# JOBR0/PerceiverIO_Pytorch

Measured on AMD Instinct MI355X. Metric: samples/sec PerceiverIO fwd (ImageNet-224, 512x1024 latents, 8 blocks x 6 self-attends), higher is better.
Workload: dtype f16; 1 GPU; imagenet224 ClassificationPerceiver (conv+Fourier prep -> encoder 3136x322->512x1024, 8x6 SA -> decoder 1000 queries -> final Linear), all rows computed; batch_per_gpu=32, global_batch=32, precision_policy=fp16x2w/fp16sd/fp16x2af, parallelism=dp1 (batch sharded, all-gather of logits), launch=one HIP graph replay per step

## Files before the change

include/pio_hip.h:

```cpp
#ifndef PIO_HIP_H
#define PIO_HIP_H

#include <stddef.h>
#include <stdint.h>

#ifdef __cplusplus
extern "C" {
#endif

#define PIO_VERSION 100

enum {
    PIO_OK = 0,
    PIO_E_SHAPE = -1,
    PIO_E_ALIGN = -2,
    PIO_E_ARCH = -3,
    PIO_E_WORKSPACE = -4,
    PIO_E_LAUNCH = -5,
    PIO_E_ARG = -6,
    PIO_E_RANGE = -7
};

enum { PIO_DT_F16 = 0, PIO_DT_BF16 = 1 };


typedef struct pio_linear_t {
    const void *w_hi;
    const void *w_lo;
    const float *bias;
    int32_t n;
    int32_t k;
    int32_t lo_row0;
} pio_linear_t;

typedef struct pio_layernorm_t {
    const float *gamma;
    const float *beta;
    int32_t c;
    float eps;
} pio_layernorm_t;

typedef struct pio_attention_t {
    pio_linear_t q, k, v, o;
    int32_t heads;
    int32_t dk, dv;
    int32_t dkp, dvp;
    int32_t q_in, k_in, v_in, out;
    int32_t dtype;
    int32_t act_split;
    pio_linear_t qk;
    pio_linear_t qkv;
    pio_linear_t kq, vo;
} pio_attention_t;

typedef struct pio_mlp_t {
    pio_linear_t fc1, fc2;
    int32_t in, hidden, out;
    int32_t dtype;
    int32_t act_split;
} pio_mlp_t;

typedef struct pio_ln_fold_t {
    pio_linear_t qkv;
    const float *qkv_c;
    pio_linear_t fc1;
    const float *fc1_c;
    int32_t *range_flag;
} pio_ln_fold_t;

typedef struct pio_self_attention_t {
    pio_layernorm_t ln1, ln2;
    pio_attention_t attn;
    pio_mlp_t mlp;
    pio_ln_fold_t fold;
} pio_self_attention_t;

typedef struct pio_cross_attention_t {
    pio_layernorm_t ln_q, ln_kv, ln2;
    pio_attention_t attn;
    pio_mlp_t mlp;
    int32_t use_query_residual;
} pio_cross_attention_t;

typedef struct pio_tensor3_t {
    const float *data;
    int64_t stride_b;
    int64_t stride_t;
    int32_t B, T, C;
} pio_tensor3_t;

int pio_version(void);
int pio_arch_ok(void);
const char *pio_error_string(int code);

#define PIO_PROF_CLASSES 9
int pio_prof_begin(int32_t max_records);
int pio_prof_end(double *ms, double *flops, double *bytes, int64_t *launches);

int pio_qk_logit_absmax(int32_t dtype, int32_t dkp, int32_t dk, const void *Q, const void *K, int32_t B, int32_t H,
                        int32_t Tq, int32_t Tk, int64_t ldq, int64_t ldk, int64_t sQb, int64_t sKb, const uint8_t *kv_mask,
                        const uint8_t *q_mask, const uint8_t *full_mask, float *absmax, void *stream);
int pio_logit_probe_begin(float *records, int32_t max_records);
int pio_logit_probe_end(void);

int pio_absmax16(int32_t dtype, const void *x, int64_t rows, int32_t cols, int64_t ld, int32_t batch, int64_t stride_b,
                 float *absmax, void *stream);
enum {
    PIO_RK_CAST = 0,
    PIO_RK_Q = 1,
    PIO_RK_K = 2,
    PIO_RK_V = 3,
    PIO_RK_ATTN = 4,
    PIO_RK_HIDDEN = 5,
    PIO_RK_STREAM = 6
};
enum { PIO_RP_ATTENTION = 0, PIO_RP_CROSS = 1, PIO_RP_STACK = 2, PIO_RP_DECODER = 3 };
int pio_range_probe_begin(float *records, int32_t max_records);
int pio_range_probe_mark(int32_t part);
int pio_range_probe_end(int32_t *parts, int32_t *kinds, int32_t cap);

int pio_ln_fold_enable(int on);

int pio_gemm_kernel_override(int which);

int pio_stream_create_cu_mask(void **stream, const uint32_t *mask, uint32_t words);
int pio_stream_destroy(void *stream);
int pio_set_cu_budget(int32_t n_cu);

int32_t pio_pad8(int32_t c);
int32_t pio_padc(int32_t c);
size_t pio_packed_weight_bytes(int32_t out, int32_t in, int32_t row_heads, int32_t col_heads);
int pio_pack_linear(const float *w, const float *bias, int32_t out, int32_t in, int64_t ldw,
                    int32_t row_heads, int32_t col_heads, void *dst_hi, void *dst_lo, float *dst_bias,
                    int32_t dst_row0, int32_t k_pad, int32_t dtype, void *stream);

int pio_layernorm_cast(const pio_tensor3_t *x, const pio_layernorm_t *ln, void *y, void *y_lo, int32_t c_pad,
                       int32_t dtype, void *stream);

int pio_layernorm_cast_cat(const pio_tensor3_t *x1, const pio_tensor3_t *x2, const pio_layernorm_t *ln, void *y,
                           void *y_lo, int32_t c_pad, int32_t dtype, void *stream);

int pio_bn_relu_maxpool_tokens(const float *x, const float *scale, const float *shift, float *y, int32_t B, int32_t C,
                               int32_t H, int32_t W, int32_t pad_top, int32_t pad_left, void *stream);

typedef struct pio_gemm_t {
    const void *A, *B;
    const void *A_lo, *B_lo;
    void *C;
    void *C_lo;
    int32_t M, N, K;
    int64_t lda, ldb, ldc;
    int32_t batch, nh;
    int64_t sAb, sAh, sBb, sBh, sCb, sCh;
    const float *bias;
    int32_t bias_mode;
    int32_t act;
    float alpha;
    const float *R;
    int64_t ldr, r_stride_b;
    int32_t r_rows_per_batch;
    int32_t out_f32;
    int32_t n_store;
    int32_t dtype;
    void *X16;
    int64_t ld16;
    float *row_part;
    const float *ln_part;
    const float *ln_c;
    float ln_eps;
    void *X16_lo;
    const void *R16_hi, *R16_lo;
    int32_t b_lo_n0;
    int32_t *range_flag;
    int32_t ln_slots;
    int32_t row_slot_w;
} pio_gemm_t;
int pio_gemm_nt(const pio_gemm_t *g, void *stream);

int pio_softmax_rows(const float *S, int64_t lds, void *P, void *P_lo, int64_t ldp, int32_t B, int32_t H,
                     int32_t Tq, int32_t Tk, float scale, const uint8_t *kv_mask, const uint8_t *q_mask,
                     const uint8_t *full_mask, const float *bias, int32_t dtype, void *stream);

int pio_flash_attention(int32_t dtype, int32_t dkp, int32_t dvp, int32_t dk, const void *Q, const void *K, const void *V,
                        void *O, int32_t B, int32_t H, int32_t Tq, int32_t Tk, int64_t ldq, int64_t ldk, int64_t ldv,
                        int64_t ldo, int64_t sQb, int64_t sKb, int64_t sVb, int64_t sOb, int32_t v_rowmajor, void *stream);

size_t pio_flash_attention_pair_workspace_bytes(int32_t dkp, int32_t dvp, int32_t B, int32_t H, int32_t Tq, int32_t Tk);
int pio_flash_attention_pair(int32_t dtype, int32_t dkp, int32_t dvp, int32_t dk, const void *Q, const void *Q_lo,
                             const void *K, const void *K_lo, const void *V, void *O, void *O_lo, int32_t B, int32_t H,
                             int32_t Tq, int32_t Tk, int64_t ldq, int64_t ldk, int64_t ldv, int64_t ldo, int64_t sQb,
                             int64_t sKb, int64_t sVb, int64_t sOb, int32_t v_rowmajor, const uint8_t *kv_mask,
                             const uint8_t *q_mask, int32_t core, void *workspace, size_t workspace_bytes, void *stream);

size_t pio_attention_workspace_bytes(const pio_attention_t *a, int32_t B, int32_t Tq, int32_t Tk);
int pio_attention_fwd(const pio_attention_t *a, const pio_tensor3_t *inputs_q, const pio_tensor3_t *inputs_k,
                      const pio_tensor3_t *inputs_v, const uint8_t *kv_mask, const uint8_t *q_mask,
                      const uint8_t *full_mask, const float *attention_bias, float *out, float *probs_out,
                      void *workspace, size_t workspace_bytes, void *stream);

size_t pio_mlp_workspace_bytes(const pio_mlp_t *m, int64_t rows);
int pio_mlp_fwd(const pio_mlp_t *m, const pio_tensor3_t *x, float *out, void *workspace,
                size_t workspace_bytes, void *stream);

typedef struct pio_call_opts_t {
    int32_t ln_fold;
    int32_t cu_budget;
} pio_call_opts_t;

size_t pio_self_attention_workspace_bytes(const pio_self_attention_t *s, int32_t B, int32_t N);
int pio_self_attention_fwd(const pio_self_attention_t *s, const pio_tensor3_t *x, const uint8_t *kv_mask,
                           const uint8_t *q_mask, const uint8_t *full_mask, const float *attention_bias,
                           float *out, float *probs_out, void *workspace, size_t workspace_bytes, void *stream);

int pio_self_attention_fwd_opts(const pio_self_attention_t *s, const pio_tensor3_t *x, const uint8_t *kv_mask,
                                const uint8_t *q_mask, const uint8_t *full_mask, const float *attention_bias,
                                float *out, float *probs_out, void *workspace, size_t workspace_bytes, void *stream,
                                const pio_call_opts_t *opts);

size_t pio_cross_attention_workspace_bytes(const pio_cross_attention_t *c, int32_t B, int32_t Tq, int32_t Tk);
int pio_cross_attention_fwd(const pio_cross_attention_t *c, const pio_tensor3_t *inputs_q,
                            const pio_tensor3_t *inputs_kv, const uint8_t *kv_mask, const uint8_t *q_mask,
                            const uint8_t *full_mask, const float *attention_bias, float *out, float *probs_out,
                            void *workspace, size_t workspace_bytes, void *stream);

size_t pio_encoder_workspace_bytes(const pio_cross_attention_t *cross, const pio_self_attention_t *layers,
                                   int32_t L, int32_t B, int32_t M, int32_t N);
int pio_encoder_fwd(const pio_cross_attention_t *cross, const pio_self_attention_t *layers, int32_t L,
                    int32_t num_blocks, const pio_tensor3_t *inputs, const pio_tensor3_t *latents,
                    const uint8_t *input_mask, float *out, void *workspace, size_t workspace_bytes,
                    void *stream);

int pio_encoder_fwd_split(const pio_cross_attention_t *cross, const pio_self_attention_t *layers, int32_t L,
                          int32_t num_blocks, const pio_tensor3_t *inputs, const pio_tensor3_t *inputs_tail,
                          const pio_tensor3_t *latents, const uint8_t *input_mask, float *out, void *workspace,
                          size_t workspace_bytes, void *stream);

int pio_encoder_fwd_blocks(const pio_cross_attention_t *cross, const pio_self_attention_t *layers, int32_t L,
                           int32_t num_blocks, int32_t per_block, const pio_tensor3_t *inputs,
                           const pio_tensor3_t *inputs_tail, const pio_tensor3_t *latents, const uint8_t *input_mask,
                           float *out, void *workspace, size_t workspace_bytes, void *stream);

int pio_encoder_fwd_opts(const pio_cross_attention_t *cross, const pio_self_attention_t *layers, int32_t L,
                         int32_t num_blocks, int32_t per_block, const pio_tensor3_t *inputs,
                         const pio_tensor3_t *inputs_tail, const pio_tensor3_t *latents, const uint8_t *input_mask,
                         float *out, void *workspace, size_t workspace_bytes, void *stream,
                         const pio_call_opts_t *opts);

size_t pio_decoder_workspace_bytes(const pio_cross_attention_t *cross, const pio_linear_t *final_layer,
                                   int32_t B, int32_t Q, int32_t N);
int pio_decoder_fwd(const pio_cross_attention_t *cross, const pio_linear_t *final_layer, int32_t final_out,
                    const pio_tensor3_t *query, const pio_tensor3_t *latents, const uint8_t *query_mask,
                    float *out, void *workspace, size_t workspace_bytes, void *stream);

size_t pio_decoder_qcache_bytes(const pio_cross_attention_t *cross, int32_t Bq, int32_t Q);
int pio_decoder_fwd_qcache(const pio_cross_attention_t *cross, const pio_linear_t *final_layer, int32_t final_out,
                           const pio_tensor3_t *query, const pio_tensor3_t *latents, const uint8_t *query_mask,
                           float *out, void *workspace, size_t workspace_bytes, void *stream, void *q16_hi,
                           void *q16_lo, int32_t q16_valid);

int pio_decoder_fwd_split(const pio_cross_attention_t *cross, const pio_linear_t *final_layer, int32_t final_out,
                          const pio_tensor3_t *query, const pio_tensor3_t *query_tail, const pio_tensor3_t *latents,
                          const uint8_t *query_mask, float *out, void *workspace, size_t workspace_bytes, void *stream);

#ifdef __cplusplus
}
#endif
#endif
```

perceiverio_pytorch_amd/_lib.py:

```python
from __future__ import annotations

import ctypes as C
import os
import subprocess

_HERE = os.path.dirname(os.path.abspath(__file__))
LIB_PATH = os.environ.get("PIO_LIB_PATH", os.path.join(_HERE, "libpio_hip.so"))
CSRC = os.path.join(_HERE, "csrc")

PIO_DT_F16 = 0
PIO_DT_BF16 = 1

PIO_OK = 0
_ERRORS = {-1: "PIO_E_SHAPE", -2: "PIO_E_ALIGN", -3: "PIO_E_ARCH", -4: "PIO_E_WORKSPACE", -5: "PIO_E_LAUNCH",
           -6: "PIO_E_ARG", -7: "PIO_E_RANGE"}


class PioError(RuntimeError):
    pass


class Linear(C.Structure):
    _fields_ = [("w_hi", C.c_void_p), ("w_lo", C.c_void_p), ("bias", C.c_void_p), ("n", C.c_int32), ("k", C.c_int32),
                ("lo_row0", C.c_int32)]


class LayerNorm(C.Structure):
    _fields_ = [("gamma", C.c_void_p), ("beta", C.c_void_p), ("c", C.c_int32), ("eps", C.c_float)]


class Attention(C.Structure):
    _fields_ = [("q", Linear), ("k", Linear), ("v", Linear), ("o", Linear), ("heads", C.c_int32),
                ("dk", C.c_int32), ("dv", C.c_int32), ("dkp", C.c_int32), ("dvp", C.c_int32),
                ("q_in", C.c_int32), ("k_in", C.c_int32), ("v_in", C.c_int32), ("out", C.c_int32), ("dtype", C.c_int32),
                ("act_split", C.c_int32), ("qk", Linear), ("qkv", Linear), ("kq", Linear), ("vo", Linear)]


class Mlp(C.Structure):
    _fields_ = [("fc1", Linear), ("fc2", Linear), ("in_", C.c_int32), ("hidden", C.c_int32), ("out", C.c_int32),
                ("dtype", C.c_int32), ("act_split", C.c_int32)]


class LnFold(C.Structure):
    _fields_ = [("qkv", Linear), ("qkv_c", C.c_void_p), ("fc1", Linear), ("fc1_c", C.c_void_p),
                ("range_flag", C.c_void_p)]


class SelfAttention(C.Structure):
    _fields_ = [("ln1", LayerNorm), ("ln2", LayerNorm), ("attn", Attention), ("mlp", Mlp), ("fold", LnFold)]


class CrossAttention(C.Structure):
    _fields_ = [("ln_q", LayerNorm), ("ln_kv", LayerNorm), ("ln2", LayerNorm), ("attn", Attention), ("mlp", Mlp),
                ("use_query_residual", C.c_int32)]


class Tensor3(C.Structure):
    _fields_ = [("data", C.c_void_p), ("stride_b", C.c_int64), ("stride_t", C.c_int64), ("B", C.c_int32),
                ("T", C.c_int32), ("C", C.c_int32)]


class CallOpts(C.Structure):
    _fields_ = [("ln_fold", C.c_int32), ("cu_budget", C.c_int32)]


class Gemm(C.Structure):
    _fields_ = [("A", C.c_void_p), ("B", C.c_void_p), ("A_lo", C.c_void_p), ("B_lo", C.c_void_p), ("C", C.c_void_p),
                ("C_lo", C.c_void_p),
                ("M", C.c_int32), ("N", C.c_int32), ("K", C.c_int32),
                ("lda", C.c_int64), ("ldb", C.c_int64), ("ldc", C.c_int64),
                ("batch", C.c_int32), ("nh", C.c_int32),
                ("sAb", C.c_int64), ("sAh", C.c_int64), ("sBb", C.c_int64), ("sBh", C.c_int64),
                ("sCb", C.c_int64), ("sCh", C.c_int64),
                ("bias", C.c_void_p), ("bias_mode", C.c_int32), ("act", C.c_int32), ("alpha", C.c_float),
                ("R", C.c_void_p), ("ldr", C.c_int64), ("r_stride_b", C.c_int64),
                ("r_rows_per_batch", C.c_int32), ("out_f32", C.c_int32), ("n_store", C.c_int32),
                ("dtype", C.c_int32),
                ("X16", C.c_void_p), ("ld16", C.c_int64), ("row_part", C.c_void_p), ("ln_part", C.c_void_p),
                ("ln_c", C.c_void_p), ("ln_eps", C.c_float),
                ("X16_lo", C.c_void_p), ("R16_hi", C.c_void_p), ("R16_lo", C.c_void_p), ("b_lo_n0", C.c_int32),
                ("range_flag", C.c_void_p), ("ln_slots", C.c_int32), ("row_slot_w", C.c_int32)]


P = C.POINTER
_vp, _i32, _i64, _sz, _f = C.c_void_p, C.c_int32, C.c_int64, C.c_size_t, C.c_float
SIGNATURES = {
    "pio_version": (C.c_int, []),
    "pio_arch_ok": (C.c_int, []),
    "pio_error_string": (C.c_char_p, [C.c_int]),
    "pio_prof_begin": (C.c_int, [_i32]),
    "pio_prof_end": (C.c_int, [P(C.c_double), P(C.c_double), P(C.c_double), P(C.c_int64)]),
    "pio_qk_logit_absmax": (C.c_int, [_i32, _i32, _i32, _vp, _vp, _i32, _i32, _i32, _i32, _i64, _i64, _i64, _i64, _vp, _vp,
                                      _vp, _vp, _vp]),
    "pio_logit_probe_begin": (C.c_int, [_vp, _i32]),
    "pio_logit_probe_end": (C.c_int, []),
    "pio_absmax16": (C.c_int, [_i32, _vp, _i64, _i32, _i64, _i32, _i64, _vp, _vp]),
    "pio_range_probe_begin": (C.c_int, [_vp, _i32]),
    "pio_range_probe_mark": (C.c_int, [_i32]),
    "pio_range_probe_end": (C.c_int, [P(_i32), P(_i32), _i32]),
    "pio_pad8": (_i32, [_i32]),
    "pio_padc": (_i32, [_i32]),
    "pio_gemm_kernel_override": (C.c_int, [C.c_int]),
    "pio_ln_fold_enable": (C.c_int, [C.c_int]),
    "pio_stream_create_cu_mask": (C.c_int, [P(_vp), P(C.c_uint32), C.c_uint32]),
    "pio_stream_destroy": (C.c_int, [_vp]),
    "pio_set_cu_budget": (C.c_int, [_i32]),
    "pio_packed_weight_bytes": (_sz, [_i32, _i32, _i32, _i32]),
    "pio_pack_linear": (C.c_int, [_vp, _vp, _i32, _i32, _i64, _i32, _i32, _vp, _vp, _vp, _i32, _i32, _i32, _vp]),
    "pio_layernorm_cast": (C.c_int, [P(Tensor3), P(LayerNorm), _vp, _vp, _i32, _i32, _vp]),
    "pio_layernorm_cast_cat": (C.c_int, [P(Tensor3), P(Tensor3), P(LayerNorm), _vp, _vp, _i32, _i32, _vp]),
    "pio_bn_relu_maxpool_tokens": (C.c_int, [_vp, _vp, _vp, _vp, _i32, _i32, _i32, _i32, _i32, _i32, _vp]),
    "pio_gemm_nt": (C.c_int, [P(Gemm), _vp]),
    "pio_softmax_rows": (C.c_int, [_vp, _i64, _vp, _vp, _i64, _i32, _i32, _i32, _i32, _f, _vp, _vp, _vp, _vp, _i32, _vp]),
    "pio_flash_attention": (C.c_int, [_i32, _i32, _i32, _i32, _vp, _vp, _vp, _vp, _i32, _i32, _i32, _i32, _i64, _i64, _i64,
                                      _i64, _i64, _i64, _i64, _i64, _i32, _vp]),
    "pio_flash_attention_pair_workspace_bytes": (_sz, [_i32, _i32, _i32, _i32, _i32, _i32]),
    "pio_flash_attention_pair": (C.c_int, [_i32, _i32, _i32, _i32, _vp, _vp, _vp, _vp, _vp, _vp, _vp, _i32, _i32, _i32, _i32,
                                           _i64, _i64, _i64, _i64, _i64, _i64, _i64, _i64, _i32, _vp, _vp, _i32, _vp, _sz,
                                           _vp]),
    "pio_attention_workspace_bytes": (_sz, [P(Attention), _i32, _i32, _i32]),
    "pio_attention_fwd": (C.c_int, [P(Attention), P(Tensor3), P(Tensor3), P(Tensor3), _vp, _vp, _vp, _vp, _vp, _vp,
                                    _vp, _sz, _vp]),
    "pio_mlp_workspace_bytes": (_sz, [P(Mlp), _i64]),
    "pio_mlp_fwd": (C.c_int, [P(Mlp), P(Tensor3), _vp, _vp, _sz, _vp]),
    "pio_self_attention_workspace_bytes": (_sz, [P(SelfAttention), _i32, _i32]),
    "pio_self_attention_fwd": (C.c_int, [P(SelfAttention), P(Tensor3), _vp, _vp, _vp, _vp, _vp, _vp, _vp, _sz, _vp]),
    "pio_self_attention_fwd_opts": (C.c_int, [P(SelfAttention), P(Tensor3), _vp, _vp, _vp, _vp, _vp, _vp, _vp, _sz, _vp,
                                              P(CallOpts)]),
    "pio_cross_attention_workspace_bytes": (_sz, [P(CrossAttention), _i32, _i32, _i32]),
    "pio_cross_attention_fwd": (C.c_int, [P(CrossAttention), P(Tensor3), P(Tensor3), _vp, _vp, _vp, _vp, _vp, _vp,
                                          _vp, _sz, _vp]),
    "pio_encoder_workspace_bytes": (_sz, [P(CrossAttention), P(SelfAttention), _i32, _i32, _i32, _i32]),
    "pio_encoder_fwd": (C.c_int, [P(CrossAttention), P(SelfAttention), _i32, _i32, P(Tensor3), P(Tensor3), _vp, _vp,
                                  _vp, _sz, _vp]),
    "pio_encoder_fwd_split": (C.c_int, [P(CrossAttention), P(SelfAttention), _i32, _i32, P(Tensor3), P(Tensor3),
                                        P(Tensor3), _vp, _vp, _vp, _sz, _vp]),
    "pio_encoder_fwd_blocks": (C.c_int, [P(CrossAttention), P(SelfAttention), _i32, _i32, _i32, P(Tensor3), P(Tensor3),
                                         P(Tensor3), _vp, _vp, _vp, _sz, _vp]),
    "pio_encoder_fwd_opts": (C.c_int, [P(CrossAttention), P(SelfAttention), _i32, _i32, _i32, P(Tensor3), P(Tensor3),
                                       P(Tensor3), _vp, _vp, _vp, _sz, _vp, P(CallOpts)]),
    "pio_decoder_workspace_bytes": (_sz, [P(CrossAttention), P(Linear), _i32, _i32, _i32]),
    "pio_decoder_fwd": (C.c_int, [P(CrossAttention), P(Linear), _i32, P(Tensor3), P(Tensor3), _vp, _vp, _vp, _sz,
                                  _vp]),
    "pio_decoder_qcache_bytes": (_sz, [P(CrossAttention), _i32, _i32]),
    "pio_decoder_fwd_qcache": (C.c_int, [P(CrossAttention), P(Linear), _i32, P(Tensor3), P(Tensor3), _vp, _vp, _vp, _sz,
                                         _vp, _vp, _vp, _i32]),
    "pio_decoder_fwd_split": (C.c_int, [P(CrossAttention), P(Linear), _i32, P(Tensor3), P(Tensor3), P(Tensor3), _vp, _vp, _vp,
                                        _sz, _vp]),
}

_lib = None


def build(verbose: bool = False) -> str:
    out = subprocess.run(["make", "-C", CSRC, "-j8"], capture_output=True, text=True)
    if verbose or out.returncode:
        print(out.stdout[-4000:])
        print(out.stderr[-4000:])
    if out.returncode:
        raise PioError("building libpio_hip.so failed")
    return LIB_PATH


def lib() -> C.CDLL:
    global _lib
    if _lib is None:
        if not os.path.exists(LIB_PATH):
            raise PioError(f"{LIB_PATH} is missing: run `python -c 'import __graft_entry__ as g; g.build()'` "
                           "(there is no CPU / eager fallback for the PerceiverIO hot path)")
        l = C.CDLL(LIB_PATH)
        for name, (res, args) in SIGNATURES.items():
            fn = getattr(l, name)
            fn.restype = res
            fn.argtypes = args
        _lib = l
    return _lib


def check(code: int, what: str = "") -> None:
    if code != PIO_OK:
        raise PioError(f"{what}: {_ERRORS.get(code, code)}")
```

perceiverio_pytorch_amd/csrc/pio_blocks.hip:

```cpp
#include "pio_internal.h"

namespace pio {

#define PIO_TRY(expr)                  \
    do {                               \
        int _e = (expr);               \
        if (_e != PIO_OK) return _e;   \
    } while (0)

#define PIO_RANGE(kind, dtype, ptr, rows, cols, ld, batch, stride_b, stream) \
    do {                                                                      \
        if (range_probe_active())                                             \
            PIO_TRY(range_probe_record(kind, dtype, ptr, rows, cols, ld, batch, stride_b, stream)); \
    } while (0)

struct Pair {
    void *hi = nullptr, *lo = nullptr;
};

static Pair take_pair(Carver &c, size_t elems, bool split) {
    Pair p;
    p.hi = c.take(elems * 2);
    p.lo = split ? c.take(elems * 2) : nullptr;
    return p;
}

struct Residual {
    const float *ptr = nullptr;
    int64_t ld = 0, stride_b = 0;
    int rows_per_batch = 0;
};

static inline int pitch4(int c) { return (c + 3) & ~3; }

static Residual residual_of(const pio_tensor3_t &t) {
    Residual r;
    r.ptr = t.data;
    r.ld = t.stride_t;
    r.stride_b = t.stride_b;
    r.rows_per_batch = t.T;
    return r;
}

static pio_gemm_t gemm_defaults(int dtype) {
    pio_gemm_t g = {};
    g.batch = 1;
    g.nh = 1;
    g.alpha = 1.f;
    g.dtype = dtype;
    return g;
}

struct LnFold {
    const float *in_part = nullptr;
    const pio_linear_t *w = nullptr;
    const float *c = nullptr;
    float eps = 0.f;
    void *out16 = nullptr;
    int64_t ld16 = 0;
    float *out_part = nullptr;
    void *out16_lo = nullptr;
    const void *res16_hi = nullptr, *res16_lo = nullptr;
    int32_t *range_flag = nullptr;
    int in_slots = 0, slot_w = 0;
};

static int linear_fwd(const pio_linear_t &lin_plain, int dtype, Pair x, int64_t rows, void *y, void *y_lo, bool out_f32,
                      int n_logical, int64_t ldc, int act, const Residual *res, hipStream_t s,
                      const LnFold *fold = nullptr, int n_store16 = 0) {
    const pio_linear_t &lin = (fold && fold->in_part) ? *fold->w : lin_plain;
    pio_gemm_t g = gemm_defaults(dtype);
    if (fold && fold->in_part) {
        g.ln_part = fold->in_part;
        g.ln_c = fold->c;
        g.ln_eps = fold->eps;
        g.ln_slots = fold->in_slots;
    }
    if (fold && fold->out16) {
        g.X16 = fold->out16;
        g.ld16 = fold->ld16;
        g.row_part = fold->out_part;
        g.X16_lo = fold->out16_lo;
        g.R16_hi = fold->res16_hi;
        g.R16_lo = fold->res16_lo;
        g.range_flag = fold->range_flag;
        g.row_slot_w = fold->slot_w;
    }
    g.A = x.hi;
    g.A_lo = x.lo;
    g.B = lin.w_hi;
    g.B_lo = lin.w_lo;
    g.b_lo_n0 = lin.w_lo ? lin.lo_row0 : 0;
    g.C = y;
    g.C_lo = y_lo;
    g.M = (int)rows;
    g.N = out_f32 ? n_logical : lin.n;
    if (out_f32 && (n_logical & 3) && ldc >= pitch4(n_logical) && lin.n >= pitch4(n_logical) &&
        !(res && res->ptr && res->ld < pitch4(n_logical)))
        g.N = pitch4(n_logical);
    g.K = lin.k;
    g.lda = lin.k;
    g.ldb = lin.k;
    g.ldc = ldc;
    g.bias = lin.bias;
    g.bias_mode = lin.bias ? 1 : 0;
    g.act = act;
    g.out_f32 = out_f32 ? 1 : 0;
    g.n_store = (!out_f32 && n_store16 > g.N) ? n_store16 : g.N;
    if (res && res->ptr && !(fold && fold->res16_hi)) {
        g.R = res->ptr;
        g.ldr = res->ld;
        g.r_stride_b = res->stride_b;
        g.r_rows_per_batch = res->rows_per_batch;
    }
    return gemm_nt_launch(g, s);
}

static int cast_pair(const pio_tensor3_t &x, const pio_layernorm_t *ln, Pair y, int c_pad, int dtype, hipStream_t s,
                     int range_kind = PIO_RK_CAST) {
    PIO_TRY(layernorm_cast_launch(x, ln, y.hi, y.lo, c_pad, dtype, s));
    PIO_RANGE(range_kind, dtype, y.hi, (int64_t)x.B * x.T, x.C, c_pad, 1, 0, s);
    return PIO_OK;
}

static const int64_t kScoreCapBytes = 1ll << 30;

struct ScoreChunks {
    int b_chunk;
    int q_chunk;
};
static ScoreChunks score_chunks(int B, int H, int Tq, int Tk) {
    const int64_t per_sample = (int64_t)H * Tq * (int64_t)Tk * 4;
    ScoreChunks c{B, Tq};
    if ((int64_t)B * per_sample <= kScoreCapBytes) return c;
    int64_t bc = kScoreCapBytes / (per_sample > 0 ? per_sample : 1);
    if (bc >= 1) {
        c.b_chunk = (int)bc;
        return c;
    }
    c.b_chunk = 1;
    int64_t qc = kScoreCapBytes / ((int64_t)H * Tk * 4);
    qc = qc / 128 * 128;
    c.q_chunk = (int)(qc < 128 ? 128 : qc);
    if (c.q_chunk > Tq) c.q_chunk = Tq;
    return c;
}

struct AttnScratch {
    Pair q16, k16, vt16, p16, o16;
    float *scores;
    void *xpart;
    void carve(Carver &c, const pio_attention_t &a, int Bq, int B, int Tq, int Tk, bool lean = false) {
        const int64_t ldq = (int64_t)a.heads * a.dkp, ldo = (int64_t)a.heads * a.dvp, tkp = pad8(Tk);
        const int64_t tkv = round_up(Tk, 32);
        const bool sp = a.act_split != 0;
        const AttnRoute plan = attn_plan(a, B, Bq, Tq, Tk, lean);
        q16 = take_pair(c, (size_t)Bq * Tq * ldq, sp);
        k16 = take_pair(c, (size_t)B * Tk * ldq, sp);
        vt16 = take_pair(c, (size_t)B * ldo * tkv, sp);
        scores = nullptr;
        p16 = Pair();
        if (plan.need_scores) {
            const ScoreChunks ch = score_chunks(B, a.heads, Tq, Tk);
            scores = (float *)c.take((size_t)ch.b_chunk * a.heads * ch.q_chunk * (int64_t)Tk * 4);
            p16 = take_pair(c, (size_t)ch.b_chunk * a.heads * ch.q_chunk * tkp, sp);
        }
        o16 = take_pair(c, (size_t)B * Tq * ldo, sp);
        xpart = plan.xpart_bytes ? c.take(plan.xpart_bytes) : nullptr;
    }
};

static int check_attention(const pio_attention_t &a) {
    if (a.heads <= 0 || a.dk <= 0 || a.dv <= 0) return PIO_E_SHAPE;
    if (a.dkp != pad8(a.dk) || a.dvp != pad8(a.dv)) return PIO_E_SHAPE;
    if (a.q.n != a.heads * a.dkp || a.k.n != a.heads * a.dkp || a.v.n != a.heads * a.dvp) return PIO_E_SHAPE;
    if (a.o.k != a.heads * a.dvp || a.q.k != padc(a.q_in) || a.k.k != padc(a.k_in) || a.v.k != padc(a.v_in))
        return PIO_E_SHAPE;
    if (!a.q.w_hi || !a.k.w_hi || !a.v.w_hi || !a.o.w_hi) return PIO_E_ARG;
    return PIO_OK;
}

static bool kv_fold_enabled() {
    const char *e = getenv("PIO_KV_FOLD");
    return !e || atoi(e) != 0;
}

struct QCache {
    Pair pair;
    bool valid;
};

static int materialised_core(const pio_attention_t &a, const AttnOperands &t, bool q_bcast, int B, int Tq, int Tk,
                             const uint8_t *kv_mask, const uint8_t *q_mask, const uint8_t *full_mask,
                             const float *attention_bias, float *probs_out, AttnScratch &w, hipStream_t s) {
    const int H = a.heads;
    const int64_t ldq = t.ldq, ldo = (int64_t)H * a.dvp, tkp = pad8(Tk), tkv = round_up(Tk, 32);
    const ScoreChunks ch = score_chunks(B, H, Tq, Tk);
    if ((full_mask || attention_bias || probs_out) && ch.q_chunk != Tq) return PIO_E_WORKSPACE;
    for (int b0 = 0; b0 < B; b0 += ch.b_chunk) {
        const int nb = b0 + ch.b_chunk <= B ? ch.b_chunk : B - b0;
        for (int r0 = 0; r0 < Tq; r0 += ch.q_chunk) {
            const int nr = r0 + ch.q_chunk <= Tq ? ch.q_chunk : Tq - r0;
            const int64_t qoff = (q_bcast ? 0 : (int64_t)b0 * Tq * ldq) + (int64_t)r0 * ldq;
            const int64_t koff = (int64_t)b0 * Tk * ldq;
            {
                pio_gemm_t g = gemm_defaults(a.dtype);
                g.A = (const char *)t.Q + qoff * 2;
                g.A_lo = t.Q_lo ? (const char *)t.Q_lo + qoff * 2 : nullptr;
                g.B = (const char *)t.K + koff * 2;
                g.B_lo = t.K_lo ? (const char *)t.K_lo + koff * 2 : nullptr;
                g.C = w.scores;
                g.M = nr;
                g.N = Tk;
                g.K = a.dkp;
                g.lda = ldq;
                g.ldb = ldq;
                g.ldc = Tk;
                g.batch = nb * H;
                g.nh = H;
                g.sAb = t.sQb;
                g.sAh = a.dkp;
                g.sBb = t.sKb;
                g.sBh = a.dkp;
                g.sCb = (int64_t)H * nr * Tk;
                g.sCh = (int64_t)nr * Tk;
                g.out_f32 = 1;
                g.n_store = Tk;
                PIO_TRY(gemm_nt_launch(g, s));
            }
            {
                const int64_t moff = (int64_t)b0 * H * Tq * Tk;
                PIO_TRY(softmax_rows_launch(w.scores, Tk, w.p16.hi, w.p16.lo, tkp, nb, H, nr, Tk,
                                            1.0f / sqrtf((float)a.dk), kv_mask ? kv_mask + (int64_t)b0 * Tk : nullptr,
                                            q_mask ? q_mask + (int64_t)b0 * Tq + r0 : nullptr,
                                            full_mask ? full_mask + (int64_t)b0 * Tq * Tk : nullptr,
                                            attention_bias ? attention_bias + moff : nullptr, a.dtype,
                                            probs_out ? probs_out + moff : nullptr, s));
            }
            {
                const int64_t ooff = ((int64_t)b0 * Tq + r0) * ldo, voff = (int64_t)b0 * ldo * tkv;
                pio_gemm_t g = gemm_defaults(a.dtype);
                g.A = w.p16.hi;
                g.A_lo = w.p16.lo;
                g.B = (const char *)w.vt16.hi + voff * 2;
                g.B_lo = w.vt16.lo ? (const char *)w.vt16.lo + voff * 2 : nullptr;
                g.C = (char *)w.o16.hi + ooff * 2;
                g.C_lo = w.o16.lo ? (char *)w.o16.lo + ooff * 2 : nullptr;
                g.M = nr;
                g.N = a.dvp;
                g.K = (int)tkp;
                g.lda = tkp;
                g.ldb = tkv;
                g.ldc = ldo;
                g.batch = nb * H;
                g.nh = H;
                g.sAb = (int64_t)H * nr * tkp;
                g.sAh = (int64_t)nr * tkp;
                g.sBb = ldo * tkv;
                g.sBh = (int64_t)a.dvp * tkv;
                g.sCb = (int64_t)Tq * ldo;
                g.sCh = a.dvp;
                g.n_store = a.dvp;
                PIO_TRY(gemm_nt_launch(g, s));
            }
        }
    }
    return PIO_OK;
}

static int attention_core(const pio_attention_t &a, Pair xq, bool q_bcast, Pair xk, Pair xv, int B, int Tq, int Tk,
                          const uint8_t *kv_mask, const uint8_t *q_mask, const uint8_t *full_mask,
                          const float *attention_bias, const Residual *res, float *out, float *probs_out,
                          AttnScratch &w, hipStream_t s, const LnFold *fold_in = nullptr,
                          const LnFold *fold_out = nullptr, int64_t out_ld = 0, const QCache *qc = nullptr) {
    if (!out_ld) out_ld = a.out;
    PIO_TRY(check_attention(a));
    if (qc) {
        if (!qc->pair.hi || (a.act_split && !qc->pair.lo)) return PIO_E_ARG;
        w.q16 = qc->pair;
    }
    const int H = a.heads;
    const int64_t hdk = (int64_t)H * a.dkp, ldo = (int64_t)H * a.dvp, ld3 = 2 * hdk + ldo, tkv = round_up(Tk, 32);
    const int Bq = q_bcast ? 1 : B;
    AttnCall call = {};
    call.B = B; call.Bq = Bq; call.Tq = Tq; call.Tk = Tk; call.q_bcast = q_bcast; call.same_qk = xq.hi == xk.hi;
    call.same_kv = xk.hi == xv.hi; call.kv_fold_on = kv_fold_enabled();
    call.kv_mask = kv_mask; call.q_mask = q_mask; call.full_mask = full_mask; call.bias = attention_bias;
    call.probs = probs_out; call.qcache = qc; call.fold_in = fold_in; call.fold_out = fold_out;
    call.fold_qkv = (fold_in && fold_in->in_part) ? fold_in->w : nullptr;
    call.qkv_adjacent = (char *)w.q16.hi < (char *)w.k16.hi && (char *)w.k16.hi < (char *)w.vt16.hi &&
                        (size_t)((char *)w.vt16.hi - (char *)w.q16.hi) + (size_t)B * ldo * tkv * 2 >= (size_t)B * Tq * ld3 * 2;
    call.qk_adjacent = (char *)w.q16.hi + (size_t)B * Tq * hdk * 2 <= (char *)w.k16.hi;
    const AttnRoute r = attn_route(a, call);
    if (r.err != PIO_OK) return r.err;
    if (r.qk_pair && (!w.q16.lo || !w.k16.lo)) return PIO_E_ARG;
    if (r.need_scores && !w.scores) return PIO_E_WORKSPACE;
    const bool kv_fold = r.core == AttnCore::KVFOLD_XATTN || r.core == AttnCore::KVFOLD_XTALL;
    const int64_t sQ = q_bcast ? 0 : 1;

    AttnOperands t = {};
    t.O = w.o16.hi;
    t.O_lo = r.out_pair ? w.o16.lo : nullptr;
    if (r.core == AttnCore::QKV_FLASH) {
        PIO_TRY(linear_fwd(a.qkv, a.dtype, xq, (int64_t)B * Tq, w.q16.hi, nullptr, false, 0, ld3, 0, nullptr, s, fold_in));
        PIO_RANGE(PIO_RK_Q, a.dtype, w.q16.hi, (int64_t)B * Tq, ld3, ld3, 1, 0, s);
        const char *base = (const char *)w.q16.hi;
        t.Q = base; t.K = base + hdk * 2; t.VT = base + 2 * hdk * 2;
        t.ldq = t.ldk = t.ldvt = ld3; t.ldo = ldo;
        t.sQb = t.sKb = t.sVb = (int64_t)Tq * ld3; t.sOb = (int64_t)Tq * ldo;
    } else if (kv_fold) {
        const int64_t kvp = a.dkp, ldx = padc(a.k_in);
        PIO_TRY(linear_fwd(a.q, a.dtype, xq, (int64_t)Bq * Tq, w.q16.hi, w.q16.lo, false, 0, hdk, 0, nullptr, s));
        PIO_RANGE(PIO_RK_Q, a.dtype, w.q16.hi, (int64_t)Bq * Tq, hdk, hdk, 1, 0, s);
        PIO_TRY(linear_fwd(a.kq, a.dtype, w.q16, (int64_t)Bq * Tq, w.k16.hi, w.k16.lo, false, 0, kvp, 0, nullptr, s));
        PIO_RANGE(PIO_RK_Q, a.dtype, w.k16.hi, (int64_t)Bq * Tq, kvp, kvp, 1, 0, s);
        PIO_TRY(transpose16_launch(xk.hi, ldx, B, Tk, (int)kvp, w.vt16.hi, tkv, s));
        t.Q = w.k16.hi; t.K = xk.hi; t.VT = w.vt16.hi;
        t.ldq = kvp; t.ldk = ldx; t.ldvt = tkv; t.ldo = kvp;
        t.sQb = sQ * Tq * kvp; t.sKb = (int64_t)Tk * ldx; t.sVb = kvp * tkv; t.sOb = (int64_t)Tq * kvp;
    } else {
        const int64_t ldq = r.fuse_qk ? 2 * hdk : hdk;
        if (r.fuse_qk) {
            PIO_TRY(linear_fwd(a.qk, a.dtype, xq, (int64_t)B * Tq, w.q16.hi, nullptr, false, 0, ldq, 0, nullptr, s));
            PIO_RANGE(PIO_RK_Q, a.dtype, w.q16.hi, (int64_t)B * Tq, ldq, ldq, 1, 0, s);
        } else {
            if (!(qc && qc->valid)) {
                PIO_TRY(linear_fwd(a.q, a.dtype, xq, (int64_t)Bq * Tq, w.q16.hi, w.q16.lo, false, 0, ldq, 0, nullptr, s));
                PIO_RANGE(PIO_RK_Q, a.dtype, w.q16.hi, (int64_t)Bq * Tq, ldq, ldq, 1, 0, s);
            }
            PIO_TRY(linear_fwd(a.k, a.dtype, xk, (int64_t)B * Tk, w.k16.hi, w.k16.lo, false, 0, ldq, 0, nullptr, s));
            PIO_RANGE(PIO_RK_K, a.dtype, w.k16.hi, (int64_t)B * Tk, ldq, ldq, 1, 0, s);
        }
        pio_gemm_t g = gemm_defaults(a.dtype);
        g.A = a.v.w_hi;
        g.A_lo = a.v.w_lo;
        g.B = xv.hi;
        g.B_lo = xv.lo;
        g.C = w.vt16.hi;
        g.C_lo = w.vt16.lo;
        g.M = a.v.n;
        g.N = Tk;
        g.K = a.v.k;
        g.lda = a.v.k;
        g.ldb = a.v.k;
        g.ldc = tkv;
        g.batch = B;
        g.sBb = (int64_t)Tk * a.v.k;
        g.sCb = ldo * tkv;
        g.bias = a.v.bias;
        g.bias_mode = a.v.bias ? 2 : 0;
        g.n_store = (int)tkv;
        PIO_TRY(gemm_nt_launch(g, s));
        PIO_RANGE(PIO_RK_V, a.dtype, w.vt16.hi, ldo, Tk, tkv, B, ldo * tkv, s);
        t.Q = w.q16.hi; t.K = r.fuse_qk ? (const char *)w.q16.hi + hdk * 2 : w.k16.hi; t.VT = w.vt16.hi;
        if (r.qk_pair) { t.Q_lo = w.q16.lo; t.K_lo = w.k16.lo; }
        t.ldq = t.ldk = ldq; t.ldvt = tkv; t.ldo = ldo;
        t.sQb = sQ * Tq * ldq; t.sKb = (int64_t)Tk * ldq; t.sVb = ldo * tkv; t.sOb = (int64_t)Tq * ldo;
    }

    if (logit_probe_active())
        PIO_TRY(logit_probe_record(a.dtype, a.dkp, a.dk, t, B, H, Tq, Tk, kv_mask, q_mask, full_mask, s));
    switch (r.core) {
    case AttnCore::QKV_FLASH: case AttnCore::PAIR_FLASH: case AttnCore::FLASH:
        PIO_TRY(flash_attention_launch(a.dtype, a.dkp, a.dvp, a.dk, t, B, H, Tq, Tk, r.core == AttnCore::QKV_FLASH, s));
        break;
    case AttnCore::KVFOLD_XATTN: case AttnCore::PAIR_XATTN: case AttnCore::XATTN:
        PIO_TRY(xattn_launch(a.dtype, a.dkp, a.dvp, a.dk, t, B, H, Tq, Tk, kv_mask, q_mask, w.xpart, s));
        break;
    case AttnCore::KVFOLD_XTALL: case AttnCore::XTALL:
        PIO_TRY(xtall_launch(a.dtype, a.dkp, a.dvp, a.dk, t, B, H, Tq, Tk, kv_mask, q_mask, w.xpart, s));
        break;
    case AttnCore::MATERIALISED:
        PIO_TRY(materialised_core(a, t, q_bcast, B, Tq, Tk, kv_mask, q_mask, full_mask, attention_bias, probs_out, w, s));
        break;
    }
    PIO_RANGE(PIO_RK_ATTN, a.dtype, w.o16.hi, (int64_t)B * Tq, t.ldo, t.ldo, 1, 0, s);
    PIO_TRY(linear_fwd(kv_fold ? a.vo : a.o, a.dtype, w.o16, (int64_t)B * Tq, out, nullptr, true, a.out, out_ld, 0, res, s,
                       fold_out));
    if (fold_out && fold_out->out16)
        PIO_RANGE(PIO_RK_STREAM, a.dtype, fold_out->out16, (int64_t)B * Tq, a.out, fold_out->ld16, 1, 0, s);
    return PIO_OK;
}

static int mlp_core(const pio_mlp_t &m, Pair x, int64_t rows, Pair h, const Residual *res, float *out,
                    hipStream_t s, const LnFold *fold_in = nullptr, const LnFold *fold_out = nullptr,
                    int64_t out_ld = 0, const Pair *out16 = nullptr) {
    if (!out_ld) out_ld = m.out;
    if (m.fc1.k != padc(m.in) || m.fc1.n != padc(m.hidden) || m.fc2.k != m.fc1.n) return PIO_E_SHAPE;
    PIO_TRY(linear_fwd(m.fc1, m.dtype, x, rows, h.hi, h.lo, false, 0, m.fc1.n, 1, nullptr, s, fold_in));
    PIO_RANGE(PIO_RK_HIDDEN, m.dtype, h.hi, rows, m.hidden, m.fc1.n, 1, 0, s);
    if (out16) {
        PIO_TRY(linear_fwd(m.fc2, m.dtype, h, rows, out16->hi, out16->lo, false, 0, padc(m.out), 0, res, s, nullptr,
                           padc(m.out)));
        PIO_RANGE(PIO_RK_STREAM, m.dtype, out16->hi, rows, m.out, padc(m.out), 1, 0, s);
        return PIO_OK;
    }
    PIO_TRY(linear_fwd(m.fc2, m.dtype, h, rows, out, nullptr, true, m.out, out_ld, 0, res, s, fold_out));
    if (fold_out && fold_out->out16)
        PIO_RANGE(PIO_RK_STREAM, m.dtype, fold_out->out16, rows, m.out, fold_out->ld16, 1, 0, s);
    return PIO_OK;
}

struct AttentionPlan {
    Pair xq16, xk16, xv16;
    AttnScratch core;
    size_t carve(void *base, const pio_attention_t &a, int B, int Tq, int Tk, bool qb, bool same) {
        Carver c(base);
        const bool sp = a.act_split != 0;
        const int Bq = qb ? 1 : B;
        xq16 = take_pair(c, (size_t)Bq * Tq * padc(a.q_in), sp);
        xk16 = take_pair(c, (size_t)B * Tk * padc(a.k_in), sp);
        xv16 = same ? xk16 : take_pair(c, (size_t)B * Tk * padc(a.v_in), sp);
        core.carve(c, a, Bq, B, Tq, Tk);
        return c.off;
    }
};

static bool same_tensor(const pio_tensor3_t &a, const pio_tensor3_t &b) {
    return a.data == b.data && a.stride_b == b.stride_b && a.stride_t == b.stride_t && a.B == b.B && a.T == b.T &&
           a.C == b.C;
}

static pio_tensor3_t first_batch(const pio_tensor3_t &t) {
    pio_tensor3_t r = t;
    r.B = 1;
    return r;
}

static Pair pair_if(Pair p, bool split) {
    if (!split) p.lo = nullptr;
    return p;
}

static bool fold_inplace() {
    const char *e = getenv("PIO_FOLD_INPLACE");
    return !e || atoi(e) != 0;
}

struct SelfPlan {
    Pair x16, h16;
    float *x1;
    AttnScratch core;
    void *x16b = nullptr, *lo_a = nullptr, *lo_b = nullptr;
    float *part_a = nullptr, *part_b = nullptr;
    size_t carve(void *base, const pio_self_attention_t &sa, int B, int N, bool lean = false) {
        Carver c(base);
        const int64_t rows = (int64_t)B * N;
        const int cmax = padc(sa.attn.q_in) > padc(sa.mlp.in) ? padc(sa.attn.q_in) : padc(sa.mlp.in);
        x16 = take_pair(c, (size_t)rows * cmax, sa.attn.act_split || sa.mlp.act_split);
        h16 = take_pair(c, (size_t)rows * padc(sa.mlp.hidden), sa.mlp.act_split != 0);
        x1 = (float *)c.take((size_t)rows * sa.attn.out * 4);
        core.carve(c, sa.attn, B, B, N, N, lean);
        if (sa.fold.qkv.w_hi && sa.fold.fc1.w_hi) {
            const bool inplace = fold_inplace();
            x16b = inplace ? x16.hi : c.take((size_t)rows * cmax * 2);
            lo_a = c.take((size_t)rows * cmax * 2);
            lo_b = inplace ? lo_a : c.take((size_t)rows * cmax * 2);
            part_a = (float *)c.take((size_t)rows * (cmax / 64 + 1) * 2 * 4);
            part_b = (float *)c.take((size_t)rows * (cmax / 64 + 1) * 2 * 4);
            if (inplace && !sa.mlp.act_split && !sa.attn.act_split &&
                (size_t)rows * padc(sa.mlp.hidden) <= (size_t)rows * sa.attn.heads * sa.attn.dvp)
                h16.hi = core.o16.hi;
        }
        return c.off;
    }
};

static int &ln_fold_global() {
    static int choice = [] {
        const char *e = getenv("PIO_LN_FOLD");
        const int v = e ? atoi(e) : 1;
        return v < 0 ? 0 : v > 2 ? 2 : v;
    }();
    return choice;
}
static thread_local int tl_ln_fold = 0;
static int ln_fold_choice() { return tl_ln_fold > 0 ? tl_ln_fold - 1 : ln_fold_global(); }
struct CallOpts {
    int prev_fold, prev_cu;
    explicit CallOpts(const pio_call_opts_t *o) : prev_fold(tl_ln_fold), prev_cu(cu_budget_call(-1)) {
        if (o) {
            tl_ln_fold = (o->ln_fold >= 0 && o->ln_fold <= 3) ? o->ln_fold : 0;
            cu_budget_call(o->cu_budget > 0 ? o->cu_budget : 0);
        }
    }
    ~CallOpts() {
        tl_ln_fold = prev_fold;
        cu_budget_call(prev_cu);
    }
};
int ln_fold_enable(int on) {
    int &c = ln_fold_global();
    const int prev = c;
    c = on < 0 ? 0 : on > 2 ? 2 : on;
    return prev;
}
bool ln_fold_enabled() { return ln_fold_choice() != 0; }
static int64_t ln_fold_min_rows() {
    static const int64_t auto_rows = [] {
        const char *e = getenv("PIO_LN_FOLD_MIN_ROWS");
        const long long v = e ? atoll(e) : 6144;
        return (int64_t)(v < 2048 ? 2048 : v);
    }();
    return ln_fold_choice() == 2 ? 2048 : auto_rows;
}
static int64_t ln_fold_small_min_rows() {
    static const int64_t auto_rows = [] {
        const char *e = getenv("PIO_LN_FOLD_SMALL_MIN_ROWS");
        const long long v = e ? atoll(e) : 512;
        return (int64_t)(v < 128 ? 128 : v);
    }();
    return ln_fold_choice() == 2 ? 128 : auto_rows;
}
static int64_t ln_fold_small_max_rows() {
    static const int64_t max_rows = [] {
        const char *e = getenv("PIO_LN_FOLD_SMALL_MAX_ROWS");
        return (int64_t)(e ? atoll(e) : 4096);
    }();
    return max_rows;
}

struct FoldCarry {
    const void *x = nullptr;
    const void *x16 = nullptr;
    const float *part = nullptr;
    bool f32_valid = true;
};

static int self_attention_run(const pio_self_attention_t &sa, const pio_tensor3_t &x, const uint8_t *kv_mask,
                              const uint8_t *q_mask, const uint8_t *full_mask, const float *attention_bias,
                              float *out, float *probs_out, SelfPlan &p, hipStream_t s, FoldCarry *carry = nullptr,
                              bool need_f32_out = true) {
    const int B = x.B, N = x.T;
    const int64_t rows = (int64_t)B * N;
    if (x.C != sa.attn.q_in || sa.attn.k_in != x.C || sa.attn.v_in != x.C || sa.attn.out != x.C ||
        sa.mlp.in != x.C || sa.mlp.out != x.C)
        return PIO_E_SHAPE;
    const bool fold_ok = ln_fold_choice() != 0 && p.x16b && x.C >= 512 && x.C <= 1536 && (x.C % 256) == 0 &&
                         x.stride_t == x.C && (B == 1 || x.stride_b == (int64_t)N * x.C) && !sa.attn.act_split &&
                         !sa.mlp.act_split && sa.attn.qkv.w_hi &&
                         (!sa.fold.qkv.w_lo || sa.fold.qkv.lo_row0 == 2 * sa.attn.heads * sa.attn.dkp) &&
                         (!sa.fold.fc1.w_lo || sa.fold.fc1.lo_row0 == 0) && flash_supported(sa.attn.dkp, sa.attn.dvp) &&
                         sa.fold.qkv.n == sa.attn.qkv.n && sa.fold.qkv.k == x.C && sa.fold.fc1.k == x.C &&
                         sa.fold.fc1.n == sa.mlp.fc1.n && sa.mlp.hidden == x.C && sa.mlp.dtype == sa.attn.dtype &&
                         !kv_mask && !q_mask && !full_mask && !attention_bias && !probs_out &&
                         (((uintptr_t)x.data) & 15) == 0;
    const bool fold_wide = fold_ok && rows >= ln_fold_min_rows();
    const bool fold_small = fold_ok && !fold_wide && rows >= ln_fold_small_min_rows() &&
                            (ln_fold_choice() == 2 || rows < ln_fold_small_max_rows()) && !sa.fold.qkv.w_lo &&
                            !sa.fold.fc1.w_lo && !sa.attn.o.w_lo && !sa.mlp.fc2.w_lo;
    const bool fold = fold_wide || fold_small;
    if (fold) {
        const int slot_w = fold_wide ? 128 : 64, nslots = x.C / slot_w;
        if (!(carry && carry->x == x.data && carry->x16 == p.x16.hi && carry->part == p.part_a)) {
            if (carry && !carry->f32_valid) return PIO_E_ARG;
            PIO_TRY(rowstats_cast_launch(x.data, rows, x.C, slot_w, p.x16.hi, p.lo_a, p.part_a, sa.attn.dtype, s));
            PIO_RANGE(PIO_RK_STREAM, sa.attn.dtype, p.x16.hi, rows, x.C, x.C, 1, 0, s);
        }
        const Pair xa = {p.x16.hi, nullptr};
        LnFold f_qkv, f_out, f_fc1, f_fc2;
        f_qkv.in_part = p.part_a; f_qkv.w = &sa.fold.qkv; f_qkv.c = sa.fold.qkv_c; f_qkv.eps = sa.ln1.eps;
        f_out.out16 = p.x16b; f_out.ld16 = x.C; f_out.out_part = p.part_b;
        f_out.out16_lo = p.lo_b; f_out.res16_hi = p.x16.hi; f_out.res16_lo = p.lo_a;
        f_out.range_flag = f_fc2.range_flag = sa.fold.range_flag;
        f_qkv.in_slots = f_fc1.in_slots = nslots;
        f_out.slot_w = f_fc2.slot_w = slot_w;
        f_fc1.in_part = p.part_b; f_fc1.w = &sa.fold.fc1; f_fc1.c = sa.fold.fc1_c; f_fc1.eps = sa.ln2.eps;
        f_fc2.out16 = p.x16.hi; f_fc2.ld16 = x.C; f_fc2.out_part = p.part_a;
        f_fc2.out16_lo = p.lo_a; f_fc2.res16_hi = p.x16b; f_fc2.res16_lo = p.lo_b;
        const Residual rx = residual_of(x);
        PIO_TRY(attention_core(sa.attn, xa, false, xa, xa, B, N, N, nullptr, nullptr, nullptr, nullptr, &rx, nullptr,
                               nullptr, p.core, s, &f_qkv, &f_out));
        pio_tensor3_t t1 = {p.x1, (int64_t)N * x.C, x.C, B, N, x.C};
        const Pair xm = {p.x16b, nullptr};
        const Residual r1 = residual_of(t1);
        PIO_TRY(mlp_core(sa.mlp, xm, rows, p.h16, &r1, need_f32_out ? out : nullptr, s, &f_fc1, &f_fc2));
        if (carry) {
            carry->x = out;
            carry->x16 = p.x16.hi;
            carry->part = p.part_a;
            carry->f32_valid = need_f32_out;
        }
        return PIO_OK;
    }
    if (carry) {
        if (!carry->f32_valid) return PIO_E_ARG;
        *carry = FoldCarry();
    }
    const Pair xa = pair_if(p.x16, sa.attn.act_split);
    PIO_TRY(cast_pair(x, &sa.ln1, xa, padc(x.C), sa.attn.dtype, s));
    const Residual rx = residual_of(x);
    PIO_TRY(attention_core(sa.attn, xa, false, xa, xa, B, N, N, kv_mask, q_mask, full_mask, attention_bias, &rx, p.x1,
                           probs_out, p.core, s));
    pio_tensor3_t t1 = {p.x1, (int64_t)N * x.C, x.C, B, N, x.C};
    const Pair xm = pair_if(p.x16, sa.mlp.act_split);
    PIO_TRY(cast_pair(t1, &sa.ln2, xm, padc(x.C), sa.mlp.dtype, s));
    const Residual r1 = residual_of(t1);
    return mlp_core(sa.mlp, xm, rows, p.h16, &r1, out, s);
}

struct CrossPlan {
    Pair q16, kv16, h16;
    float *x1;
    AttnScratch core;
    bool q_bcast;
    size_t carve(void *base, const pio_cross_attention_t &ca, int B, int Tq, int Tk, bool qb, bool lean = false) {
        Carver c(base);
        q_bcast = qb;
        const int Bq = qb ? 1 : B;
        const int64_t rows = (int64_t)B * Tq;
        const bool sp = ca.attn.act_split || ca.mlp.act_split;
        q16 = take_pair(c, (size_t)rows * padc(ca.attn.q_in), sp);
        kv16 = take_pair(c, (size_t)B * Tk * padc(ca.attn.k_in), ca.attn.act_split != 0);
        h16 = take_pair(c, (size_t)rows * padc(ca.mlp.hidden), ca.mlp.act_split != 0);
        x1 = (float *)c.take((size_t)rows * pitch4(ca.attn.out) * 4);
        core.carve(c, ca.attn, Bq, B, Tq, Tk, lean);
        return c.off;
    }
};

static int cross_attention_run(const pio_cross_attention_t &ca, const pio_tensor3_t &iq, const pio_tensor3_t &ikv,
                               const uint8_t *kv_mask, const uint8_t *q_mask, const uint8_t *full_mask,
                               const float *attention_bias, float *out, float *probs_out, CrossPlan &p,
                               hipStream_t s, const pio_tensor3_t *ikv_tail = nullptr, int64_t out_ld = 0,
                               const QCache *qc = nullptr, const Pair *out16 = nullptr,
                               const pio_tensor3_t *iq_tail = nullptr) {
    const int B = iq.B, Tq = iq.T, Tk = ikv.T;
    const int64_t rows = (int64_t)B * Tq;
    const int kv_c = ikv.C + (ikv_tail ? ikv_tail->C : 0);
    const int q_c = iq.C + (iq_tail ? iq_tail->C : 0);
    if (q_c != ca.attn.q_in || kv_c != ca.attn.k_in || kv_c != ca.attn.v_in || ikv.B != B) return PIO_E_SHAPE;
    if (ca.attn.out != q_c || ca.mlp.in != q_c || ca.mlp.out != q_c) return PIO_E_SHAPE;
    if (iq_tail && (ca.use_query_residual || qc || p.q_bcast)) return PIO_E_ARG;
    if (ikv_tail) {
        PIO_TRY(layernorm_cast_cat_launch(ikv, *ikv_tail, ca.ln_kv, p.kv16.hi, p.kv16.lo, padc(kv_c), ca.attn.dtype, s));
        PIO_RANGE(PIO_RK_CAST, ca.attn.dtype, p.kv16.hi, (int64_t)B * Tk, kv_c, padc(kv_c), 1, 0, s);
    } else
        PIO_TRY(cast_pair(ikv, &ca.ln_kv, p.kv16, padc(ikv.C), ca.attn.dtype, s));
    const pio_tensor3_t q1 = p.q_bcast ? first_batch(iq) : iq;
    const Pair qa = pair_if(p.q16, ca.attn.act_split);
    if (qc && ca.use_query_residual) return PIO_E_ARG;
    if (iq_tail) {
        PIO_TRY(layernorm_cast_cat_launch(iq, *iq_tail, ca.ln_q, qa.hi, qa.lo, padc(q_c), ca.attn.dtype, s));
        PIO_RANGE(PIO_RK_CAST, ca.attn.dtype, qa.hi, rows, q_c, padc(q_c), 1, 0, s);
    } else if (!(qc && qc->valid)) PIO_TRY(cast_pair(q1, &ca.ln_q, qa, padc(q_c), ca.attn.dtype, s));
    const Residual rq = residual_of(iq);
    PIO_TRY(attention_core(ca.attn, qa, p.q_bcast, p.kv16, p.kv16, B, Tq, Tk, kv_mask, q_mask, full_mask,
                           attention_bias, ca.use_query_residual ? &rq : nullptr, p.x1, probs_out, p.core, s, nullptr,
                           nullptr, pitch4(q_c), qc));
    pio_tensor3_t t1 = {p.x1, (int64_t)Tq * pitch4(q_c), pitch4(q_c), B, Tq, q_c};
    const Pair qm = pair_if(p.q16, ca.mlp.act_split);
    PIO_TRY(cast_pair(t1, &ca.ln2, qm, padc(q_c), ca.mlp.dtype, s));
    const Residual r1 = residual_of(t1);
    return mlp_core(ca.mlp, qm, rows, p.h16, &r1, out, s, nullptr, nullptr, out_ld, out16);
}

struct RangePart {
    bool changed = false;
    int prev = 0;
    void set(int part) {
        if (!range_probe_active()) return;
        const int was = range_probe_mark(part);
        if (!changed) prev = was;
        changed = true;
    }
    ~RangePart() {
        if (changed) range_probe_mark(prev);
    }
};

struct DecoderPlan {
    CrossPlan cp;
    float *y;
    Pair y16;
    size_t carve(void *base, const pio_cross_attention_t &cross, const pio_linear_t *fin, int B, int Q, int N,
                 bool qb) {
        Carver c(base);
        const int64_t rows = (int64_t)B * Q;
        y = nullptr;
        y16 = Pair();
        if (fin) {
            y = (float *)c.take((size_t)rows * pitch4(cross.attn.q_in) * 4);
            y16 = take_pair(c, (size_t)rows * padc(cross.attn.q_in), cross.mlp.act_split != 0);
        }
        const size_t inner = cp.carve(base ? (char *)base + c.off : nullptr, cross, B, Q, N, qb, true);
        return c.off + inner;
    }
};

}

using namespace pio;

extern "C" {

size_t pio_attention_workspace_bytes(const pio_attention_t *a, int32_t B, int32_t Tq, int32_t Tk) {
    if (!a) return 0;
    AttentionPlan p;
    return p.carve(nullptr, *a, B, Tq, Tk, false, false);
}

int pio_attention_fwd(const pio_attention_t *a, const pio_tensor3_t *iq, const pio_tensor3_t *ik,
                      const pio_tensor3_t *iv, const uint8_t *kv_mask, const uint8_t *q_mask,
                      const uint8_t *full_mask, const float *attention_bias, float *out, float *probs_out,
                      void *workspace, size_t workspace_bytes, void *stream) {
    if (!a || !iq || !ik || !iv || !out || !workspace) return PIO_E_ARG;
    hipStream_t s = (hipStream_t)stream;
    if (iq->C != a->q_in || ik->C != a->k_in || iv->C != a->v_in) return PIO_E_SHAPE;
    if (ik->B != iq->B || iv->B != iq->B || ik->T != iv->T) return PIO_E_SHAPE;
    const int B = iq->B, Tq = iq->T, Tk = ik->T;
    const bool qb = (iq->stride_b == 0 && B > 1);
    const bool same = same_tensor(*ik, *iv);
    AttentionPlan p;
    if (p.carve(workspace, *a, B, Tq, Tk, qb, same) > workspace_bytes) return PIO_E_WORKSPACE;
    const pio_tensor3_t q1 = qb ? first_batch(*iq) : *iq;
    PIO_TRY(cast_pair(q1, nullptr, p.xq16, padc(a->q_in), a->dtype, s));
    PIO_TRY(cast_pair(*ik, nullptr, p.xk16, padc(a->k_in), a->dtype, s));
    if (!same) PIO_TRY(cast_pair(*iv, nullptr, p.xv16, padc(a->v_in), a->dtype, s));
    return attention_core(*a, p.xq16, qb, p.xk16, p.xv16, B, Tq, Tk, kv_mask, q_mask, full_mask, attention_bias,
                          nullptr, out, probs_out, p.core, s);
}

size_t pio_mlp_workspace_bytes(const pio_mlp_t *m, int64_t rows) {
    if (!m) return 0;
    Carver c(nullptr);
    take_pair(c, (size_t)rows * padc(m->in), m->act_split != 0);
    take_pair(c, (size_t)rows * padc(m->hidden), m->act_split != 0);
    return c.off;
}

int pio_mlp_fwd(const pio_mlp_t *m, const pio_tensor3_t *x, float *out, void *workspace, size_t workspace_bytes,
                void *stream) {
    if (!m || !x || !out || !workspace) return PIO_E_ARG;
    if (x->C != m->in) return PIO_E_SHAPE;
    const int64_t rows = (int64_t)x->B * x->T;
    if (pio_mlp_workspace_bytes(m, rows) > workspace_bytes) return PIO_E_WORKSPACE;
    hipStream_t s = (hipStream_t)stream;
    Carver c(workspace);
    const Pair x16 = take_pair(c, (size_t)rows * padc(m->in), m->act_split != 0);
    const Pair h16 = take_pair(c, (size_t)rows * padc(m->hidden), m->act_split != 0);
    PIO_TRY(cast_pair(*x, nullptr, x16, padc(m->in), m->dtype, s));
    return mlp_core(*m, x16, rows, h16, nullptr, out, s);
}

int pio_ln_fold_enable(int on) { return ln_fold_enable(on); }

size_t pio_self_attention_workspace_bytes(const pio_self_attention_t *sa, int32_t B, int32_t N) {
    if (!sa) return 0;
    SelfPlan p;
    return p.carve(nullptr, *sa, B, N);
}

int pio_self_attention_fwd(const pio_self_attention_t *sa, const pio_tensor3_t *x, const uint8_t *kv_mask,
                           const uint8_t *q_mask, const uint8_t *full_mask, const float *attention_bias, float *out,
                           float *probs_out, void *workspace, size_t workspace_bytes, void *stream) {
    return pio_self_attention_fwd_opts(sa, x, kv_mask, q_mask, full_mask, attention_bias, out, probs_out, workspace,
                                       workspace_bytes, stream, nullptr);
}

int pio_self_attention_fwd_opts(const pio_self_attention_t *sa, const pio_tensor3_t *x, const uint8_t *kv_mask,
                                const uint8_t *q_mask, const uint8_t *full_mask, const float *attention_bias,
                                float *out, float *probs_out, void *workspace, size_t workspace_bytes, void *stream,
                                const pio_call_opts_t *opts) {
    if (!sa || !x || !out || !workspace) return PIO_E_ARG;
    CallOpts scope(opts);
    SelfPlan p;
    if (p.carve(workspace, *sa, x->B, x->T) > workspace_bytes) return PIO_E_WORKSPACE;
    return self_attention_run(*sa, *x, kv_mask, q_mask, full_mask, attention_bias, out, probs_out, p,
                              (hipStream_t)stream);
}

size_t pio_cross_attention_workspace_bytes(const pio_cross_attention_t *ca, int32_t B, int32_t Tq, int32_t Tk) {
    if (!ca) return 0;
    CrossPlan p;
    return p.carve(nullptr, *ca, B, Tq, Tk, false);
}

int pio_cross_attention_fwd(const pio_cross_attention_t *ca, const pio_tensor3_t *iq, const pio_tensor3_t *ikv,
                            const uint8_t *kv_mask, const uint8_t *q_mask, const uint8_t *full_mask,
                            const float *attention_bias, float *out, float *probs_out, void *workspace,
                            size_t workspace_bytes, void *stream) {
    if (!ca || !iq || !ikv || !out || !workspace) return PIO_E_ARG;
    CrossPlan p;
    const bool qb = (iq->stride_b == 0 && iq->B > 1);
    if (p.carve(workspace, *ca, iq->B, iq->T, ikv->T, qb) > workspace_bytes) return PIO_E_WORKSPACE;
    return cross_attention_run(*ca, *iq, *ikv, kv_mask, q_mask, full_mask, attention_bias, out, probs_out, p,
                               (hipStream_t)stream);
}

size_t pio_encoder_workspace_bytes(const pio_cross_attention_t *cross, const pio_self_attention_t *layers, int32_t L,
                                   int32_t B, int32_t M, int32_t N) {
    if (!cross) return 0;
    CrossPlan cp;
    size_t need = cp.carve(nullptr, *cross, B, N, M, false, true);
    for (int l = 0; l < L; ++l) {
        SelfPlan sp;
        const size_t n = sp.carve(nullptr, layers[l], B, N, true);
        if (n > need) need = n;
    }
    return need;
}

int pio_encoder_fwd(const pio_cross_attention_t *cross, const pio_self_attention_t *layers, int32_t L,
                    int32_t num_blocks, const pio_tensor3_t *inputs, const pio_tensor3_t *latents,
                    const uint8_t *input_mask, float *out, void *workspace, size_t workspace_bytes, void *stream) {
    return pio_encoder_fwd_split(cross, layers, L, num_blocks, inputs, nullptr, latents, input_mask, out, workspace,
                                 workspace_bytes, stream);
}

int pio_encoder_fwd_split(const pio_cross_attention_t *cross, const pio_self_attention_t *layers, int32_t L,
                          int32_t num_blocks, const pio_tensor3_t *inputs, const pio_tensor3_t *inputs_tail,
                          const pio_tensor3_t *latents, const uint8_t *input_mask, float *out, void *workspace,
                          size_t workspace_bytes, void *stream) {
    return pio_encoder_fwd_blocks(cross, layers, L, num_blocks, 0, inputs, inputs_tail, latents, input_mask, out,
                                  workspace, workspace_bytes, stream);
}

int pio_encoder_fwd_blocks(const pio_cross_attention_t *cross, const pio_self_attention_t *layers, int32_t L,
                           int32_t num_blocks, int32_t per_block, const pio_tensor3_t *inputs,
                           const pio_tensor3_t *inputs_tail, const pio_tensor3_t *latents, const uint8_t *input_mask,
                           float *out, void *workspace, size_t workspace_bytes, void *stream) {
    return pio_encoder_fwd_opts(cross, layers, L, num_blocks, per_block, inputs, inputs_tail, latents, input_mask, out,
                                workspace, workspace_bytes, stream, nullptr);
}

int pio_encoder_fwd_opts(const pio_cross_attention_t *cross, const pio_self_attention_t *layers, int32_t L,
                         int32_t num_blocks, int32_t per_block, const pio_tensor3_t *inputs,
                         const pio_tensor3_t *inputs_tail, const pio_tensor3_t *latents, const uint8_t *input_mask,
                         float *out, void *workspace, size_t workspace_bytes, void *stream,
                         const pio_call_opts_t *opts) {
    if (!cross || !inputs || !latents || !out || !workspace || (L > 0 && !layers)) return PIO_E_ARG;
    CallOpts scope(opts);
    if (L < 0 || num_blocks < 0) return PIO_E_SHAPE;
    hipStream_t s = (hipStream_t)stream;
    const int B = inputs->B, M = inputs->T, N = latents->T, D = latents->C;
    if (latents->B != B) return PIO_E_SHAPE;
    if (pio_encoder_workspace_bytes(cross, layers, L, B, M, N) > workspace_bytes) return PIO_E_WORKSPACE;
    RangePart range_part;
    {
        CrossPlan cp;
        const bool qb = (latents->stride_b == 0 && B > 1);
        cp.carve(workspace, *cross, B, N, M, qb, true);
        PIO_TRY(cross_attention_run(*cross, *latents, *inputs, input_mask, nullptr, nullptr, nullptr, out, nullptr,
                                    cp, s, inputs_tail));
    }
    const pio_tensor3_t z = {out, (int64_t)N * D, D, B, N, D};
    range_part.set(PIO_RP_STACK);
    FoldCarry carry;
    for (int blk = 0; blk < num_blocks; ++blk) {
        for (int l = 0; l < L; ++l) {
            const pio_self_attention_t &lay = layers[(per_block ? (size_t)blk * L : 0) + l];
            SelfPlan sp;
            sp.carve(workspace, lay, B, N, true);
            const bool last = blk == num_blocks - 1 && l == L - 1;
            PIO_TRY(self_attention_run(lay, z, nullptr, nullptr, nullptr, nullptr, out, nullptr, sp, s, &carry, last));
        }
    }
    return PIO_OK;
}

size_t pio_decoder_workspace_bytes(const pio_cross_attention_t *cross, const pio_linear_t *final_layer, int32_t B,
                                   int32_t Q, int32_t N) {
    if (!cross) return 0;
    DecoderPlan p;
    return p.carve(nullptr, *cross, final_layer, B, Q, N, false);
}

int pio_decoder_fwd(const pio_cross_attention_t *cross, const pio_linear_t *final_layer, int32_t final_out,
                    const pio_tensor3_t *query, const pio_tensor3_t *latents, const uint8_t *query_mask, float *out,
                    void *workspace, size_t workspace_bytes, void *stream) {
    return pio_decoder_fwd_qcache(cross, final_layer, final_out, query, latents, query_mask, out, workspace,
                                  workspace_bytes, stream, nullptr, nullptr, 0);
}

size_t pio_decoder_qcache_bytes(const pio_cross_attention_t *cross, int32_t Bq, int32_t Q) {
    if (!cross || Bq <= 0 || Q <= 0) return 0;
    return (size_t)round_up((int64_t)Bq * Q * cross->attn.heads * cross->attn.dkp * 2, 256);
}

static int decoder_run(const pio_cross_attention_t *cross, const pio_linear_t *final_layer, int32_t final_out,
                       const pio_tensor3_t *query, const pio_tensor3_t *query_tail, const pio_tensor3_t *latents,
                       const uint8_t *query_mask, float *out, void *workspace, size_t workspace_bytes, void *stream,
                       void *q16_hi, void *q16_lo, int32_t q16_valid) {
    if (!cross || !query || !latents || !out || !workspace) return PIO_E_ARG;
    const int q_c = query->C + (query_tail ? query_tail->C : 0);
    QCache qcache{{q16_hi, q16_lo}, q16_valid != 0};
    const QCache *qc = q16_hi ? &qcache : nullptr;
    if (qc && (((uintptr_t)q16_hi & 15) || ((uintptr_t)q16_lo & 15))) return PIO_E_ALIGN;
    hipStream_t s = (hipStream_t)stream;
    const int B = query->B, Q = query->T, N = latents->T;
    if (latents->B != B) return PIO_E_SHAPE;
    DecoderPlan p;
    const bool qb = (query->stride_b == 0 && B > 1);
    if (p.carve(workspace, *cross, final_layer, B, Q, N, qb) > workspace_bytes) return PIO_E_WORKSPACE;
    float *y = final_layer ? p.y : out;
    const int64_t y_ld = final_layer ? pitch4(q_c) : q_c;
    static const bool y16_direct = [] {
        const char *e = getenv("PIO_DEC_Y16");
        return !e || atoi(e) != 0;
    }();
    const bool direct = final_layer && y16_direct && final_layer->k == padc(q_c);
    PIO_TRY(cross_attention_run(*cross, *query, *latents, nullptr, query_mask, nullptr, nullptr, y, nullptr, p.cp,
                                s, nullptr, y_ld, qc, direct ? &p.y16 : nullptr, query_tail));
    if (!final_layer) return PIO_OK;
    if (final_layer->k != padc(q_c)) return PIO_E_SHAPE;
    const pio_tensor3_t ty = {y, (int64_t)Q * y_ld, y_ld, B, Q, q_c};
    if (!direct) PIO_TRY(cast_pair(ty, nullptr, p.y16, padc(q_c), cross->attn.dtype, s, PIO_RK_STREAM));
    return linear_fwd(*final_layer, cross->attn.dtype, p.y16, (int64_t)B * Q, out, nullptr, true, final_out, final_out,
                      0, nullptr, s);
}

int pio_decoder_fwd_qcache(const pio_cross_attention_t *cross, const pio_linear_t *final_layer, int32_t final_out,
                           const pio_tensor3_t *query, const pio_tensor3_t *latents, const uint8_t *query_mask,
                           float *out, void *workspace, size_t workspace_bytes, void *stream, void *q16_hi,
                           void *q16_lo, int32_t q16_valid) {
    return decoder_run(cross, final_layer, final_out, query, nullptr, latents, query_mask, out, workspace,
                       workspace_bytes, stream, q16_hi, q16_lo, q16_valid);
}

int pio_decoder_fwd_split(const pio_cross_attention_t *cross, const pio_linear_t *final_layer, int32_t final_out,
                          const pio_tensor3_t *query, const pio_tensor3_t *query_tail, const pio_tensor3_t *latents,
                          const uint8_t *query_mask, float *out, void *workspace, size_t workspace_bytes, void *stream) {
    if (!query_tail) return PIO_E_ARG;
    return decoder_run(cross, final_layer, final_out, query, query_tail, latents, query_mask, out, workspace,
                       workspace_bytes, stream, nullptr, nullptr, 0);
}

}
```

perceiverio_pytorch_amd/perceiver.py:

```python
from __future__ import annotations

import ctypes as C
import os

import torch
import torch.nn as nn

from . import _lib as L
from . import probe as LP
from . import runtime as R
from .position_encoding import TrainablePositionEncoding
from .transformer_primitives import CrossAttention, SelfAttention, lecun_normal_, make_cross_attention_mask


class PerceiverEncoder(nn.Module):

    def __init__(self, num_input_channels: int, num_self_attends_per_block: int = 6, num_blocks: int = 8,
                 num_latents: int = 512, num_latent_channels: int = 1024, qk_channels: int = None,
                 v_channels: int = None, num_cross_attend_heads: int = 1, num_self_attend_heads: int = 8,
                 cross_attend_widening_factor: int = 1, self_attend_widening_factor: int = 1,
                 dropout_prob: float = 0.0, latent_pos_enc_init_scale: float = 0.02,
                 cross_attention_shape_for_attn: str = "kv", use_query_residual: bool = True):
        super().__init__()
        if num_latent_channels % num_self_attend_heads != 0:
            raise ValueError(f"num_z_channels ({num_latent_channels}) must be divisible by"
                             f" num_self_attend_heads ({num_self_attend_heads}).")
        if num_latent_channels % num_cross_attend_heads != 0:
            raise ValueError(f"num_z_channels ({num_latent_channels}) must be divisible by"
                             f" num_cross_attend_heads ({num_cross_attend_heads}).")
        self._num_blocks = num_blocks
        self.latent_pos_enc = TrainablePositionEncoding(index_dim=num_latents, num_channels=num_latent_channels,
                                                        init_scale=latent_pos_enc_init_scale)
        self.cross_attend = CrossAttention(q_in_channels=num_latent_channels, kv_in_channels=num_input_channels,
                                           dropout_prob=dropout_prob, num_heads=num_cross_attend_heads,
                                           widening_factor=cross_attend_widening_factor,
                                           shape_for_attn=cross_attention_shape_for_attn, qk_channels=qk_channels,
                                           v_channels=v_channels, use_query_residual=use_query_residual)
        self.self_attends = nn.ModuleList()
        for _ in range(num_self_attends_per_block):
            self.self_attends.append(SelfAttention(in_channels=num_latent_channels, num_heads=num_self_attend_heads,
                                                   dropout_prob=dropout_prob, qk_channels=qk_channels,
                                                   v_channels=v_channels,
                                                   widening_factor=self_attend_widening_factor))

    cross_attend_policy = None

    def latents(self, inputs):
        return self.latent_pos_enc(batch_size=inputs.shape[0])

    def forward(self, inputs, latents, *, input_mask=None):
        if R.cpu_plumbing(inputs[0] if isinstance(inputs, (tuple, list)) else inputs, "PerceiverEncoder.forward"):
            from . import cpu_plumbing as CP
            return CP.encoder(self, inputs, latents, input_mask)
        inputs_tail = None
        if isinstance(inputs, (tuple, list)):
            inputs, inputs_tail = inputs
            inputs_tail = R.as_f32_3d(inputs_tail if inputs_tail.dim() == 3 else inputs_tail[None])
        R.require_device(inputs, "PerceiverEncoder.forward")
        if self.training and any(m.dropout.p > 0 for m in self.self_attends):
            raise NotImplementedError("the HIP path is forward/inference only")
        lib = L.lib()
        x, z0 = R.as_f32_3d(inputs), R.as_f32_3d(latents)
        B, M, _ = x.shape
        N, D = z0.shape[1], z0.shape[2]
        dev = x.device
        with R.precision(self.cross_attend_policy):
            cross = self.cross_attend._desc()
        Lyr = len(self.self_attends)
        per_block = R.policy_block_feedback() and self._num_blocks > 1 and Lyr > 0
        nset = self._num_blocks if per_block else 1
        descs = []
        for sa in self.self_attends:
            descs.append(sa._desc_blocks(self._num_blocks) if per_block else [sa._desc()])
        im, im_ptr = R.mask_u8(input_mask, (B, M), dev)
        out = torch.empty((B, N, D), dtype=torch.float32, device=dev)
        tail3 = R.tensor3(inputs_tail) if inputs_tail is not None else None
        guard = R.range_check() and Lyr > 0 and not self._range_fallback
        flag = None
        if guard:
            flag = R.range_flag(dev, self)
            flag.zero_()
        lkey = (tuple(id(d) for ds in descs for d in ds), flag.data_ptr() if guard else 0)
        lc = self.__dict__.get("_layers_cache")
        if lc is None or lc[0] != lkey:
            layers = (L.SelfAttention * max(Lyr * nset, 1))()
            for i, ds in enumerate(descs):
                for b, d in enumerate(ds):
                    layers[b * Lyr + i] = d
            if guard:
                for i in range(Lyr * nset):
                    layers[i].fold.range_flag = flag.data_ptr()
            self.__dict__["_layers_cache"] = lc = (lkey, layers, descs)
        layers = lc[1]
        nsplit = R.batch_streams()
        if nsplit <= 1 or B < 2 * nsplit or B % nsplit or inputs_tail is not None or per_block:
            ws = R.workspace(dev, lib.pio_encoder_workspace_bytes(cross, layers, Lyr, B, M, N))
            opts = L.CallOpts(1 if self._range_fallback else 0, 0)
            LP.expect("cross", *["stack"] * (Lyr * self._num_blocks))
            LP.mark_range("cross")
            try:
                with R.on_device(dev):
                    L.check(lib.pio_encoder_fwd_opts(cross, layers, Lyr, self._num_blocks, int(per_block), R.tensor3(x),
                                                     tail3, R.tensor3(z0), im_ptr, out.data_ptr(), ws.data_ptr(),
                                                     ws.numel(), R.stream_ptr(dev), opts), "pio_encoder_fwd")
            finally:
                LP.mark_range("attention")
            return self._finish(out, flag, inputs, inputs_tail, latents, input_mask)
        cur = torch.cuda.current_stream(dev)
        bs = B // nsplit
        masked = (R.cu_split() or os.environ.get("PIO_CU_BUDGET_ONLY") == "1") and 32 % nsplit == 0
        opts = L.CallOpts(1 if self._range_fallback else 0, R.cu_share(nsplit) if masked else 0)
        sides = R.side_streams(dev, nsplit)
        for side in sides:
            side.wait_stream(cur)
        for i, side in enumerate(sides):
            LP.expect("cross", *["stack"] * (Lyr * self._num_blocks))
            LP.mark_range("cross")
            try:
                with R.on_device(dev), torch.cuda.stream(side):
                    xs, zs = x[i * bs:(i + 1) * bs], z0[i * bs:(i + 1) * bs]
                    ws = R.workspace(dev, lib.pio_encoder_workspace_bytes(cross, layers, Lyr, bs, M, N))
                    mp = im_ptr + i * bs * M if im_ptr is not None else None
                    L.check(lib.pio_encoder_fwd_opts(cross, layers, Lyr, self._num_blocks, 0, R.tensor3(xs), None,
                                                     R.tensor3(zs), mp, out[i * bs:(i + 1) * bs].data_ptr(),
                                                     ws.data_ptr(), ws.numel(), side.cuda_stream, opts), "pio_encoder_fwd")
            finally:
                LP.mark_range("attention")
        for side in sides:
            cur.wait_stream(side)
        for t in (x, z0, out):
            for side in R.side_streams(dev, nsplit):
                t.record_stream(side)
        return self._finish(out, flag, inputs, inputs_tail, latents, input_mask)

    _range_fallback = False

    def _finish(self, out, flag, inputs, inputs_tail, latents, input_mask):
        if self._range_fallback:
            if not bool(torch.isfinite(out).all()):
                raise L.PioError("PerceiverEncoder.forward: PIO_E_RANGE -- non-finite latents with and without the "
                                 "LayerNorm fold: activations exceed the fp16 operand range (65504); use the "
                                 "precision policy 'bf16x3' for this model")
        elif flag is not None and not R.capturing(out.device):
            pend = R.range_deferred()
            if pend is not None:
                pend.append(flag)
            elif int(flag.item()) != 0:
                full = inputs if inputs_tail is None else (inputs, inputs_tail)
                return self.forward_unfolded(full, latents, input_mask=input_mask)
        return R.forward_only(out, inputs, latents, *self.parameters())

    def forward_unfolded(self, inputs, latents, *, input_mask=None):
        self._range_fallback = True
        try:
            return self.forward(inputs, latents, input_mask=input_mask)
        finally:
            self._range_fallback = False


class PerceiverDecoder(nn.Module):

    def __init__(self, query_channels: int, final_project_out_channels: int, num_latent_channels: int = 1024,
                 qk_channels: int = None, v_channels: int = None, use_query_residual: bool = False,
                 output_w_init: str = "lecun_normal", num_heads: int = 1, final_project: bool = True):
        super().__init__()
        self._output_num_channels = final_project_out_channels
        self._output_w_init = output_w_init
        self._use_query_residual = use_query_residual
        self._qk_channels = qk_channels
        self._v_channels = v_channels
        self._final_project = final_project
        self._num_heads = num_heads
        self.query_channels = query_channels
        self.decoding_cross_attn = CrossAttention(q_in_channels=query_channels, kv_in_channels=num_latent_channels,
                                                  dropout_prob=0.0, num_heads=self._num_heads, widening_factor=1,
                                                  shape_for_attn="kv", qk_channels=self._qk_channels,
                                                  v_channels=self._v_channels,
                                                  use_query_residual=self._use_query_residual)
        self._final_cache = None
        if self._final_project:
            self.final_layer = nn.Linear(query_channels, self._output_num_channels)
            if self._output_w_init == "lecun_normal":
                lecun_normal_(self.final_layer.weight)
            elif self._output_w_init == "zeros":
                nn.init.constant_(self.final_layer.weight, 0)
            else:
                raise ValueError(f"{self._output_w_init} not supported as output_w_init")
            nn.init.constant_(self.final_layer.bias, 0)

    def _apply(self, fn, *a, **k):
        self._final_cache = None
        return super()._apply(fn, *a, **k)

    def _load_from_state_dict(self, *a, **k):
        self._final_cache = None
        return super()._load_from_state_dict(*a, **k)

    def _final_desc(self):
        key = R.param_key(self.final_layer.weight, self.final_layer.bias)
        if self._final_cache is None or self._final_cache[0] != key:
            dtype, wlevel, _split = R.policy_dtype()
            two = wlevel >= 2 or "final_layer" in R.policy_fine_split()
            self._final_cache = (key, R.PackedLinear(self.final_layer.weight, self.final_layer.bias, 1, 1, dtype, two))
        return self._final_cache[1]

    def forward(self, query, latents, *, query_mask=None, q_cache=None):
        query_tail = None
        if isinstance(query, (tuple, list)):
            query, query_tail = query
            if self._use_query_residual:
                raise ValueError("a (features, table) query needs use_query_residual=False")
        if R.cpu_plumbing(query, "PerceiverDecoder.forward"):
            from . import cpu_plumbing as CP
            if query_tail is not None:
                t = query_tail if query_tail.dim() == 3 else query_tail[None]
                query = torch.cat([query, t.expand(query.shape[0], -1, -1)], dim=-1)
            return CP.decoder(self, query, latents, query_mask)
        R.require_device(query, "PerceiverDecoder.forward")
        lib = L.lib()
        q, z = R.as_f32_3d(query), R.as_f32_3d(latents)
        if query_tail is not None:
            query_tail = R.as_f32_3d(query_tail if query_tail.dim() == 3 else query_tail[None])
        B, Q, _ = q.shape
        N = z.shape[1]
        dev = q.device
        cross = self.decoding_cross_attn._desc()
        fin = self._final_desc() if self._final_project else None
        out_ch = self._output_num_channels if self._final_project else self.query_channels
        qm, qm_ptr = R.mask_u8(query_mask, (B, Q), dev)
        out = torch.empty((B, Q, out_ch), dtype=torch.float32, device=dev)
        fin_ptr = C.byref(fin.desc) if fin is not None else None
        ws = R.workspace(dev, lib.pio_decoder_workspace_bytes(cross, fin_ptr, B, Q, N))
        qhi = qlo = None
        valid = 0
        if q_cache is not None and not self._use_query_residual and query_tail is None:
            ca = self.decoding_cross_attn
            Bq = 1 if (q.stride(0) == 0 and B > 1) else B
            try:
                qver = q._version
            except RuntimeError:
                qver = -1
            key = (R.param_key(ca.layer_norm_q.weight, ca.layer_norm_q.bias, ca.attention.proj_q.weight,
                               ca.attention.proj_q.bias), Bq, Q, q.data_ptr(), qver, int(cross.attn.act_split))
            fresh = q_cache.get("key") != key
            if not (R.capturing(dev) and (fresh or not q_cache.get("valid"))):
                if fresh:
                    nb = lib.pio_decoder_qcache_bytes(cross, Bq, Q)
                    with torch.inference_mode(False):
                        q_cache["hi"] = torch.empty(nb, dtype=torch.uint8, device=dev)
                        q_cache["lo"] = torch.empty(nb, dtype=torch.uint8, device=dev) if cross.attn.act_split else None
                    q_cache["key"], q_cache["valid"] = key, False
                qhi = q_cache["hi"].data_ptr()
                qlo = q_cache["lo"].data_ptr() if q_cache["lo"] is not None else None
                valid = 1 if q_cache["valid"] else 0
        LP.expect("decoder")
        LP.mark_range("decoder")
        try:
            with R.on_device(dev):
                if query_tail is not None:
                    L.check(lib.pio_decoder_fwd_split(cross, fin_ptr, out_ch, R.tensor3(q), R.tensor3(query_tail),
                                                      R.tensor3(z), qm_ptr, out.data_ptr(), ws.data_ptr(), ws.numel(),
                                                      R.stream_ptr(dev)), "pio_decoder_fwd_split")
                else:
                    L.check(lib.pio_decoder_fwd_qcache(cross, fin_ptr, out_ch, R.tensor3(q), R.tensor3(z), qm_ptr,
                                                       out.data_ptr(), ws.data_ptr(), ws.numel(), R.stream_ptr(dev), qhi,
                                                       qlo, valid), "pio_decoder_fwd")
        finally:
            LP.mark_range("attention")
        if qhi is not None:
            q_cache["valid"] = True
        return R.forward_only(out, query, latents, *self.parameters())


def restructure(modality_sizes, inputs: torch.Tensor):
    out, start = {}, 0
    for name in sorted(modality_sizes.keys()):
        n = modality_sizes[name]
        out[name] = inputs[:, start:start + n]
        start += n
    return out


def _as_module_dict(x):
    if type(x) is dict:
        return nn.ModuleDict(x)
    if isinstance(x, nn.Module) and not isinstance(x, nn.ModuleDict):
        return nn.ModuleDict({"__default": x})
    return x


class MultimodalPreprocessor(nn.Module):

    def __init__(self, input_preprocessors=None, mask_probs=None, min_padding_size: int = 2, input_channels=None):
        super().__init__()
        self._preprocessors = input_preprocessors
        self._min_padding_size = min_padding_size
        self._mask_probs = mask_probs
        if input_preprocessors is not None:
            assert input_channels is None, "input_channels and modalities are mutually exclusive"
            input_channels = {m: p.n_output_channels() for m, p in input_preprocessors.items()}
        else:
            assert input_channels is not None, "if no preprocessors, input_channels must be specified"
        self._common_channels = max(input_channels.values()) + min_padding_size
        if mask_probs is not None:
            self.mask_tokens = nn.ModuleDict({
                m: TrainablePositionEncoding(index_dim=1, num_channels=self._common_channels, init_scale=0.02)
                for m in self._preprocessors.keys()})
        self.padding_embeddings = None
        ragged = max(input_channels.values()) != min(input_channels.values())
        if ragged or min_padding_size != 0:
            self.padding_embeddings = nn.ModuleDict({
                m: TrainablePositionEncoding(index_dim=1, num_channels=self._common_channels - p.n_output_channels(),
                                             init_scale=0.02)
                for m, p in self._preprocessors.items()})

    def n_output_channels(self):
        return self._common_channels

    def forward(self, inputs, *, pos=None):
        if self._preprocessors is None:
            outputs, without_pos = inputs, inputs
        else:
            outputs, without_pos = {}, {}
            for m, prep in self._preprocessors.items():
                outputs[m], without_pos[m] = prep(inputs[m], pos=pos)
        if self.padding_embeddings is not None:
            padded = {}
            for m, x in outputs.items():
                pad = torch.broadcast_to(self.padding_embeddings[m](x.shape[0]),
                                         [x.shape[0], x.shape[1], self._common_channels - x.shape[2]])
                padded[m] = torch.cat([x, pad], dim=2)
            outputs = padded
        sizes = {m: x.shape[1] for m, x in outputs.items()}
        if self._mask_probs is not None:
            masked = {}
            for m, x in outputs.items():
                token = self.mask_tokens[m](x.shape[0])
                p = self._mask_probs[m]
                if p <= 0.0:
                    masked[m] = x
                elif p >= 1.0:
                    masked[m] = torch.broadcast_to(token, x.shape) + 0 * x
                else:
                    mask = torch.bernoulli(torch.full([x.shape[0], x.shape[1]], fill_value=float(p))).to(x.device)
                    mask = mask[:, :, None]
                    masked[m] = (1 - mask) * x + mask * token
            outputs = masked
        ordered = [outputs[m] for m in sorted(outputs.keys())]
        return torch.cat(ordered, dim=1), sizes, without_pos


class PerceiverIO(nn.Module):

    def __init__(self, num_blocks: int = 8, num_self_attends_per_block: int = 6, num_latents: int = 512,
                 num_latent_channels: int = 1024, final_project: bool = True, final_project_out_channels: int = None,
                 perceiver_encoder_kwargs=None, perceiver_decoder_kwargs=None, input_preprocessors=None,
                 output_postprocessors=None, output_queries=None, output_query_padding_channels: int = 0,
                 input_padding_channels: int = 0, input_channels=None, input_mask_probs: dict = None):
        super().__init__()
        perceiver_encoder_kwargs = perceiver_encoder_kwargs or {}
        perceiver_decoder_kwargs = perceiver_decoder_kwargs or {}
        if final_project_out_channels is None:
            final_project_out_channels = num_latent_channels
        if type(input_channels) is int:
            input_channels = {"__default": input_channels}
        self._multi_preprocessor = MultimodalPreprocessor(input_preprocessors=_as_module_dict(input_preprocessors),
                                                          mask_probs=input_mask_probs,
                                                          min_padding_size=input_padding_channels,
                                                          input_channels=input_channels)
        self._output_postprocessors = _as_module_dict(output_postprocessors)
        self._output_queries = _as_module_dict(output_queries)
        query_channels = max(q.n_query_channels() for q in self._output_queries.values()) + \
            output_query_padding_channels
        self.query_channels = query_channels
        self.padding_embeddings = nn.ModuleDict({
            m: TrainablePositionEncoding(index_dim=1, num_channels=query_channels - q.n_query_channels(),
                                         init_scale=0.02)
            for m, q in self._output_queries.items()})
        self._encoder = PerceiverEncoder(num_input_channels=self._multi_preprocessor.n_output_channels(),
                                         num_blocks=num_blocks,
                                         num_self_attends_per_block=num_self_attends_per_block,
                                         num_latents=num_latents, num_latent_channels=num_latent_channels,
                                         **perceiver_encoder_kwargs)
        self._decoder = PerceiverDecoder(query_channels=query_channels, final_project=final_project,
                                         final_project_out_channels=final_project_out_channels,
                                         num_latent_channels=num_latent_channels, **perceiver_decoder_kwargs)
        self.decoder_query_rows = None
        self.encoder_policy = None
        self.decoder_policy = None

    split_encoder_input = True

    def _split_input(self, inputs, pos):
        mp = self._multi_preprocessor
        if (pos is not None or mp._preprocessors is None or list(mp._preprocessors.keys()) != ["__default"]
                or mp.padding_embeddings is not None or mp._mask_probs is not None):
            return None
        prep = mp._preprocessors["__default"]
        if not hasattr(prep, "forward_split") or not inputs["__default"].is_cuda:
            return None
        if any(getattr(q, "_concat_preprocessed_input", False) for q in self._output_queries.values()):
            if not self._identity_query():
                return None
        return prep.forward_split(inputs["__default"])

    def _identity_query(self):
        qs = list(self._output_queries.values())
        if len(qs) != 1 or list(self._output_queries.keys()) != ["__default"]:
            return False
        q = qs[0]
        return (getattr(q, "_position_encoding", 0) is None and getattr(q, "_concat_preprocessed_input", False)
                and not self._decoder._use_query_residual and self.decoder_query_rows is None
                and q.n_query_channels() == self.query_channels)

    def decoder_query(self, inputs, modality_sizes, inputs_without_pos=None, subsampled_points=None):
        per_mod = restructure(modality_sizes, inputs)
        subsampled_points = subsampled_points or {}
        any_input = next(iter(per_mod.values()))
        queries = {}
        for m, make_query in self._output_queries.items():
            wo = inputs_without_pos.get(m) if inputs_without_pos is not None else None
            src = per_mod.get(m)
            if src is None:
                src = torch.zeros((any_input.shape[0], 0), device=any_input.device)
            q = make_query(src, inputs_without_pos=wo, subsampled_points=subsampled_points.get(m))
            q = q.reshape(q.shape[0], -1, q.shape[-1])
            pad = torch.broadcast_to(self.padding_embeddings[m](q.shape[0]),
                                     [q.shape[0], q.shape[1], self.query_channels - q.shape[2]])
            queries[m] = torch.cat([q, pad], dim=2) if pad.shape[2] > 0 else q
        sizes = {m: q.shape[1] for m, q in queries.items()}
        if len(queries) == 1:
            return next(iter(queries.values())), sizes
        return torch.cat([queries[m] for m in sorted(queries.keys())], dim=1), sizes

    def forward(self, inputs, *, subsampled_output_points=None, pos=None, input_mask=None, query_mask=None,
                query_shard=None):
        kw = dict(subsampled_output_points=subsampled_output_points, pos=pos, input_mask=input_mask,
                  query_mask=query_mask, query_shard=query_shard)
        with R.defer_range_checks() as guard:
            outputs = self._forward(inputs, **kw)
        if guard.pending and any(int(f.item()) != 0 for f in guard.pending):
            self._encoder._range_fallback = True
            try:
                outputs = self._forward(inputs, **kw)
            finally:
                self._encoder._range_fallback = False
        return outputs

    def _forward(self, inputs, *, subsampled_output_points=None, pos=None, input_mask=None, query_mask=None,
                 query_shard=None):
        if type(inputs) is torch.Tensor:
            inputs = {"__default": inputs}
        split = self._split_input(inputs, pos) if self.split_encoder_input else None
        if split is not None and split[0] == "full":
            x = split[1]
            sizes, without_pos = {"__default": x.shape[1]}, {"__default": split[2]}
            latents0 = self._encoder.latents(x)
            query, query_sizes = self.decoder_query(x, sizes, without_pos, subsampled_points=subsampled_output_points)
            with R.precision(self.encoder_policy):
                latents = self._encoder(x, latents0, input_mask=input_mask)
        elif split is not None:
            feats, table = split[1], split[2]
            sizes, without_pos = {"__default": feats.shape[1]}, {"__default": feats}
            latents0 = self._encoder.latents(feats)
            if self._identity_query() and subsampled_output_points is None and query_shard is None:
                query, query_sizes = (feats, table), dict(sizes)
            else:
                if self._identity_query():
                    x = torch.cat([feats, torch.broadcast_to(table[None], (feats.shape[0],) + tuple(table.shape))], -1)
                    query, query_sizes = self.decoder_query(x, sizes, without_pos,
                                                            subsampled_points=subsampled_output_points)
                else:
                    query, query_sizes = self.decoder_query(feats, sizes, without_pos,
                                                            subsampled_points=subsampled_output_points)
            with R.precision(self.encoder_policy):
                latents = self._encoder((feats, table), latents0, input_mask=input_mask)
        else:
            x, sizes, without_pos = self._multi_preprocessor(inputs, pos=pos)
            latents0 = self._encoder.latents(x)
            query, query_sizes = self.decoder_query(x, sizes, without_pos, subsampled_points=subsampled_output_points)
            with R.precision(self.encoder_policy):
                latents = self._encoder(x, latents0, input_mask=input_mask)
        if self.decoder_query_rows is not None:
            query = query[:, self.decoder_query_rows]
            if query_mask is not None:
                query_mask = query_mask[:, self.decoder_query_rows]
            assert len(query_sizes) == 1, "decoder_query_rows is defined for a single output modality"
            query_sizes = {m: query.shape[1] for m in query_sizes}
        with R.precision(self.decoder_policy):
            if query_shard is not None:
                from .dist import decode_query_sharded
                outputs = decode_query_sharded(self._decoder, query, latents, query_mask, *query_shard)
            else:
                outputs = self._decoder(query, latents, query_mask=query_mask)
        if self._output_postprocessors:
            per_mod = restructure(query_sizes, outputs)
            with R.precision(self.decoder_policy):
                outputs = {m: post(per_mod[m], pos=None, modality_sizes=None)
                           for m, post in self._output_postprocessors.items()}
        if type(outputs) is not torch.Tensor and list(outputs.keys()) == ["__default"]:
            outputs = outputs["__default"]
        return outputs
```

perceiverio_pytorch_amd/runtime.py:

```python
from __future__ import annotations

import ctypes as C
import os
from typing import Dict, Optional, Tuple

import torch

from . import _lib as L

_POLICIES = {"fp16": (L.PIO_DT_F16, 0, False), "fp16x2s": (L.PIO_DT_F16, 1, False),
             "fp16x2w": (L.PIO_DT_F16, 2, False), "fp16x3": (L.PIO_DT_F16, 3, True),
             "bf16": (L.PIO_DT_BF16, 0, False), "bf16x2w": (L.PIO_DT_BF16, 2, False),
             "bf16x3": (L.PIO_DT_BF16, 3, True),
             "fp16x3f": (L.PIO_DT_F16, 3, True), "bf16x3f": (L.PIO_DT_BF16, 3, True),
             "fp16x3fq": (L.PIO_DT_F16, 3, True),
             "fp16x2af": (L.PIO_DT_F16, 0, True),
             "fp16sd": (L.PIO_DT_F16, 0, False),
             "fp16x2o": (L.PIO_DT_F16, 0, False), "fp16x2v": (L.PIO_DT_F16, 0, False),
             "fp16x2afo": (L.PIO_DT_F16, 0, True)}
_FINE_SPLIT = {"fp16x2o": {"final"}, "fp16x2v": {"proj_v"}, "fp16x2afo": {"final", "final_layer", "post"}}
_FUSED_CORE = {"fp16x3f", "bf16x3f", "fp16x2af", "fp16x2afo", "fp16x3fq"}
_PAIR_CORE = {"fp16x3fq"}
_BLOCK_FEEDBACK = {"fp16sd"}
_policy = os.environ.get("PIO_PRECISION", "fp16x3")
if _policy not in _POLICIES:
    raise ValueError(f"PIO_PRECISION={_policy!r} not in {sorted(_POLICIES)}")


def set_precision_policy(name: str) -> None:
    global _policy
    if name not in _POLICIES:
        raise ValueError(f"unknown precision policy {name!r}; choose from {sorted(_POLICIES)}")
    _policy = name


def get_precision_policy() -> str:
    return _policy


class precision:

    def __init__(self, name: Optional[str]):
        if name is not None and name not in _POLICIES:
            raise ValueError(f"unknown precision policy {name!r}; choose from {sorted(_POLICIES)}")
        self._name = name
        self._saved = None

    def __enter__(self):
        global _policy
        self._saved = _policy
        if self._name is not None:
            _policy = self._name
        return self

    def __exit__(self, *exc):
        global _policy
        _policy = self._saved
        return False


def policy_dtype(name: Optional[str] = None) -> Tuple[int, bool, bool]:
    return _POLICIES[name or _policy]


_range_check = os.environ.get("PIO_RANGE_CHECK", "1") != "0"
_range_flags: Dict[tuple, torch.Tensor] = {}
_range_deferred: Optional[list] = None


def range_check() -> bool:
    return _range_check


def set_range_check(on: bool) -> None:
    global _range_check
    _range_check = bool(on)


def range_flag(device: torch.device, owner=None) -> torch.Tensor:
    idx = device.index if device.index is not None else torch.cuda.current_device()
    key = (idx, id(owner) if owner is not None else 0)
    t = _range_flags.get(key)
    if t is None:
        with torch.inference_mode(False):
            t = torch.zeros(1, dtype=torch.int32, device=device)
        _range_flags[key] = t
        if owner is not None:
            import weakref
            weakref.finalize(owner, _range_flags.pop, key, None)
    _range_flags[(idx, "last")] = t
    return t


def last_range_flag(device: Optional[torch.device] = None) -> Optional[torch.Tensor]:
    idx = (device.index if device is not None and device.index is not None else torch.cuda.current_device())
    return _range_flags.get((idx, "last"))


class defer_range_checks:

    def __enter__(self):
        global _range_deferred
        self._saved = _range_deferred
        _range_deferred = []
        self.pending = _range_deferred
        return self

    def __exit__(self, *exc):
        global _range_deferred
        _range_deferred = self._saved
        return False


def range_deferred() -> Optional[list]:
    return _range_deferred


def capturing(device: torch.device) -> bool:
    try:
        return bool(torch.cuda.is_current_stream_capturing())
    except Exception:
        return False


def policy_fine_split(name: Optional[str] = None) -> set:
    extra = set(os.environ.get("PIO_EXTRA_SPLIT", "").split(",")) - {""}
    return _FINE_SPLIT.get(name or _policy, set()) | extra


def policy_core_single(name: Optional[str] = None) -> bool:
    return (name or _policy) in _FUSED_CORE


def policy_core_pair(name: Optional[str] = None) -> bool:
    return (name or _policy) in _PAIR_CORE


def attention_act_split(name: Optional[str] = None) -> int:
    if not _POLICIES[name or _policy][2]:
        return 0
    return 3 if policy_core_pair(name) else 2 if policy_core_single(name) else 1


def policy_block_feedback(name: Optional[str] = None) -> bool:
    return (name or _policy) in _BLOCK_FEEDBACK


def feedback_images(w: torch.Tensor, nblk: int, dtype: int):
    tdt = torch.float16 if dtype == L.PIO_DT_F16 else torch.bfloat16
    w = w.detach().float()
    out, e = [], torch.zeros_like(w)
    for _ in range(nblk):
        t = w + e
        hi = t.to(tdt).float()
        e = t - hi
        out.append(hi)
    return out


def pad8(c: int) -> int:
    return (c + 7) & ~7


def padc(c: int) -> int:
    return int(L.lib().pio_padc(int(c)))


_backend = os.environ.get("PIO_BACKEND", "hip")
if _backend not in ("hip", "torch"):
    raise ValueError(f"PIO_BACKEND={_backend!r}: 'hip' or 'torch'")


def set_backend(name: str) -> None:
    global _backend
    if name not in ("hip", "torch"):
        raise ValueError(f"unknown backend {name!r}: 'hip' (MI355X kernels) or 'torch' (opt-in CPU plumbing)")
    _backend = name


def get_backend() -> str:
    return _backend


def cpu_plumbing(t: torch.Tensor, what: str) -> bool:
    if _backend != "torch":
        return False
    if t.is_cuda:
        raise L.PioError(f"{what}: backend 'torch' is the CPU plumbing path and got a {t.device} tensor; GPU tensors run "
                         "on the HIP kernels only -- set_backend('hip')")
    return True


def require_device(t: torch.Tensor, what: str) -> None:
    if not t.is_cuda:
        raise L.PioError(f"{what}: perceiverio_pytorch_amd computes on an MI355X (HIP) device only; got a "
                         f"{t.device} tensor. There is no CPU or eager fallback (an explicit CPU plumbing backend "
                         "exists for machines without a GPU: perceiverio_pytorch_amd.set_backend('torch')).")


def stream_ptr(device) -> int:
    return torch.cuda.current_stream(device).cuda_stream


def as_f32_3d(t: torch.Tensor) -> torch.Tensor:
    if t.dim() != 3:
        raise ValueError(f"expected a [B, T, C] tensor, got {tuple(t.shape)}")
    if t.dtype != torch.float32:
        t = t.float()
    if t.stride(2) != 1 and t.shape[2] != 1:
        t = t.contiguous()
    if t.stride(1) < t.shape[2] and t.shape[1] > 1:
        t = t.contiguous()
    return t


def tensor3(t: torch.Tensor) -> L.Tensor3:
    B, T, Cc = t.shape
    sb = t.stride(0) if B > 1 else T * Cc
    st = t.stride(1) if T > 1 else Cc
    return L.Tensor3(t.data_ptr(), sb, st, B, T, Cc)


def mask_u8(m: Optional[torch.Tensor], shape, device) -> Tuple[Optional[torch.Tensor], Optional[int]]:
    if m is None:
        return None, None
    if tuple(m.shape) != tuple(shape):
        raise ValueError(f"mask shape {tuple(m.shape)} != {tuple(shape)}")
    mm = m.to(device=device)
    mm = (mm != 0) if mm.dtype != torch.bool else mm
    mm = mm.contiguous().view(torch.uint8)
    return mm, mm.data_ptr()


_workspaces: Dict[Tuple[int, int], torch.Tensor] = {}


def workspace(device: torch.device, nbytes: int) -> torch.Tensor:
    key = (device.index if device.index is not None else torch.cuda.current_device(), stream_ptr(device))
    ws = _workspaces.get(key)
    if ws is None or ws.numel() < nbytes:
        ws = None
        _workspaces.pop(key, None)
        ws = torch.empty(int(nbytes * 1.05) + 4096, dtype=torch.uint8, device=device)
        _workspaces[key] = ws
    return ws


def release_workspaces() -> None:
    _workspaces.clear()


_nstreams = max(1, int(os.environ.get("PIO_STREAMS", "1")))
_side_streams: Dict[Tuple[int, int], list] = {}


def batch_streams() -> int:
    return _nstreams


def set_batch_streams(n: int) -> None:
    global _nstreams
    _nstreams = max(1, int(n))


_cu_split = os.environ.get("PIO_CU_SPLIT", "0") == "1"


def cu_split() -> bool:
    return _cu_split


def set_cu_split(on: bool) -> None:
    global _cu_split
    _cu_split = bool(on)
    release_side_streams()


_masked_cache: Dict[Tuple[int, int], list] = {}


def release_side_streams() -> None:
    _side_streams.clear()


def cu_share(n: int) -> int:
    try:
        total = torch.cuda.get_device_properties(torch.cuda.current_device()).multi_processor_count
    except Exception:
        total = 256
    return total // n


def _masked_streams(device: torch.device, n: int) -> list:
    import ctypes as C
    lib = L.lib()
    per = 32 // n
    out = []
    for i in range(n):
        words = (C.c_uint32 * 8)()
        for j in range(256):
            if i * per <= j // 8 < (i + 1) * per:
                words[j // 32] |= 1 << (j % 32)
        h = C.c_void_p()
        with torch.cuda.device(device):
            L.check(lib.pio_stream_create_cu_mask(C.byref(h), words, 8), "pio_stream_create_cu_mask")
        out.append(torch.cuda.ExternalStream(h.value, device=device))
    return out


def side_streams(device: torch.device, n: int) -> list:
    key = (device.index if device.index is not None else torch.cuda.current_device(), n, _cu_split)
    if key not in _side_streams:
        if _cu_split and 32 % n == 0:
            mk = (key[0], n)
            if mk not in _masked_cache:
                _masked_cache[mk] = _masked_streams(device, n)
            _side_streams[key] = _masked_cache[mk]
        else:
            _side_streams[key] = [torch.cuda.Stream(device=device) for _ in range(n)]
    return _side_streams[key]


class PackedLinear:

    def __init__(self, weight: torch.Tensor, bias: Optional[torch.Tensor], row_heads: int, col_heads: int,
                 dtype: int, two_pass: bool, *, k_channels: bool = True, n_channels: bool = False):
        require_device(weight, "pack_linear")
        lib = L.lib()
        out, inn = weight.shape
        if out % row_heads or inn % col_heads:
            raise ValueError("channels must be divisible by the head count")
        rows_packed = row_heads * pad8(out // row_heads)
        self.n = padc(out) if (n_channels and row_heads == 1) else rows_packed
        self.k = padc(inn) if (k_channels and col_heads == 1) else col_heads * pad8(inn // col_heads)
        dev = weight.device
        w = weight.detach()
        if w.dtype != torch.float32 or not w.is_contiguous():
            w = w.float().contiguous()
        tdt = torch.float16 if dtype == L.PIO_DT_F16 else torch.bfloat16
        alloc = torch.zeros if self.n > rows_packed else torch.empty
        self.hi = alloc((self.n, self.k), dtype=tdt, device=dev)
        self.lo = alloc((self.n, self.k), dtype=tdt, device=dev) if two_pass else None
        self.bias = alloc((self.n,), dtype=torch.float32, device=dev)
        b = None
        if bias is not None:
            b = bias.detach()
            if b.dtype != torch.float32 or not b.is_contiguous():
                b = b.float().contiguous()
        L.check(lib.pio_pack_linear(w.data_ptr(), b.data_ptr() if b is not None else None, out, inn, inn,
                                    row_heads, col_heads, self.hi.data_ptr(),
                                    self.lo.data_ptr() if two_pass else None, self.bias.data_ptr(), 0, self.k,
                                    dtype, stream_ptr(dev)), "pio_pack_linear")
        self.desc = L.Linear(self.hi.data_ptr(), self.lo.data_ptr() if two_pass else None, self.bias.data_ptr(),
                             self.n, self.k)


class PackedStack:

    def __init__(self, pairs, row_heads: int, dtype: int, two_pass):
        lib = L.lib()
        flags = [bool(two_pass)] * len(pairs) if isinstance(two_pass, bool) else [bool(f) for f in two_pass]
        if any(a and not b for a, b in zip(flags, flags[1:])):
            raise ValueError("only a suffix of the stacked linears may be split")
        two_pass = any(flags)
        w0 = pairs[0][0]
        require_device(w0, "pack_linear")
        dev = w0.device
        inn = w0.shape[1]
        self.k = padc(inn)
        rows = [row_heads * pad8(w.shape[0] // row_heads) for w, _ in pairs]
        self.n = sum(rows)
        tdt = torch.float16 if dtype == L.PIO_DT_F16 else torch.bfloat16
        self.hi = torch.empty((self.n, self.k), dtype=tdt, device=dev)
        self.lo = torch.empty((self.n, self.k), dtype=tdt, device=dev) if two_pass else None
        self.bias = torch.empty((self.n,), dtype=torch.float32, device=dev)
        if self.lo is not None and not all(flags):
            self.lo.zero_()
        r0 = 0
        lo_row0 = 0
        for (w, b), nr, fl in zip(pairs, rows, flags):
            if w.shape[1] != inn:
                raise ValueError("stacked linears need equal in_features")
            wf = w.detach().float().contiguous()
            bf = b.detach().float().contiguous() if b is not None else None
            L.check(lib.pio_pack_linear(wf.data_ptr(), bf.data_ptr() if bf is not None else None, w.shape[0], inn,
                                        inn, row_heads, 1, self.hi.data_ptr(),
                                        self.lo.data_ptr() if fl else None, self.bias.data_ptr(), r0, self.k,
                                        dtype, stream_ptr(dev)), "pio_pack_linear")
            if not fl:
                lo_row0 = r0 + nr
            r0 += nr
        self.lo_row0 = lo_row0 if two_pass else 0
        self.desc = L.Linear(self.hi.data_ptr(), self.lo.data_ptr() if two_pass else None, self.bias.data_ptr(),
                             self.n, self.k, self.lo_row0)


def _version_of(p: torch.Tensor) -> int:
    return 0 if p.is_inference() else p._version


def param_key(*params) -> tuple:
    return tuple((p.data_ptr(), _version_of(p), str(p.device)) if p is not None else None for p in params) + (_policy,)


def invalidate_packed_weights(module: torch.nn.Module) -> None:
    for m in module.modules():
        if hasattr(m, "_pio_cache"):
            m._pio_cache = None
        if hasattr(m, "_pio_block_cache"):
            m._pio_block_cache = None
        if hasattr(m, "_final_cache"):
            m._final_cache = None


class _ForwardOnly(torch.autograd.Function):

    @staticmethod
    def forward(ctx, out, *deps):
        return out.view_as(out)

    @staticmethod
    def backward(ctx, *grads):
        raise NotImplementedError("perceiverio_pytorch_amd is a forward / inference path: there is no backward "
                                  "through the HIP kernels (run under torch.inference_mode() or torch.no_grad())")


def forward_only(out: torch.Tensor, *deps) -> torch.Tensor:
    if torch.is_grad_enabled():
        live = [t for t in deps if isinstance(t, torch.Tensor) and t.requires_grad]
        if live:
            return _ForwardOnly.apply(out, *live)
    return out


class on_device:

    def __init__(self, device: torch.device):
        self._ctx = torch.cuda.device(device)

    def __enter__(self):
        self._ctx.__enter__()
        return self

    def __exit__(self, *exc):
        return self._ctx.__exit__(*exc)


def layernorm_desc(ln: torch.nn.LayerNorm, keep: list) -> L.LayerNorm:
    w, b = ln.weight.detach(), ln.bias.detach()
    if w.dtype != torch.float32:
        w, b = w.float(), b.float()
    w, b = w.contiguous(), b.contiguous()
    keep += [w, b]
    return L.LayerNorm(w.data_ptr(), b.data_ptr(), w.numel(), float(ln.eps))


def hip_linear(x: torch.Tensor, weight: torch.Tensor, bias: Optional[torch.Tensor], cache: dict) -> torch.Tensor:
    import ctypes as C
    require_device(x, "hip_linear")
    lib = L.lib()
    dev = x.device
    dtype, wlevel, split = policy_dtype()
    key = param_key(weight, bias)
    pk = cache.get("packed")
    if pk is None or pk[0] != key:
        pk = (key, PackedLinear(weight, bias, 1, 1, dtype, wlevel >= 2 or "post" in policy_fine_split()))
        cache["packed"] = pk
    lin = pk[1]
    lead = x.shape[:-1]
    x3 = as_f32_3d(x.reshape(1, -1, x.shape[-1]))
    rows, n_out = x3.shape[1], weight.shape[0]
    tdt = torch.float16 if dtype == L.PIO_DT_F16 else torch.bfloat16
    x16 = torch.empty((rows, lin.k), dtype=tdt, device=dev)
    x16lo = torch.empty((rows, lin.k), dtype=tdt, device=dev) if split else None
    out = torch.empty((rows, n_out), dtype=torch.float32, device=dev)
    with on_device(dev):
        L.check(lib.pio_layernorm_cast(tensor3(x3), None, x16.data_ptr(), x16lo.data_ptr() if split else None, lin.k,
                                       dtype, stream_ptr(dev)), "pio_layernorm_cast")
        g = L.Gemm()
        g.A, g.B = x16.data_ptr(), lin.hi.data_ptr()
        g.A_lo = x16lo.data_ptr() if split else None
        g.B_lo = lin.lo.data_ptr() if lin.lo is not None else None
        g.C = out.data_ptr()
        g.M, g.N, g.K = rows, n_out, lin.k
        g.lda = g.ldb = lin.k
        g.ldc = n_out
        g.batch = g.nh = 1
        g.bias = lin.bias.data_ptr()
        g.bias_mode = 1
        g.alpha = 1.0
        g.out_f32 = 1
        g.n_store = n_out
        g.dtype = dtype
        L.check(lib.pio_gemm_nt(C.byref(g), stream_ptr(dev)), "pio_gemm_nt")
    return forward_only(out.reshape(lead + (n_out,)), x, weight, bias)
```

perceiverio_pytorch_amd/transformer_primitives.py:

```python
from __future__ import annotations

import math
import os
from typing import Optional

import torch
import torch.nn as nn

from . import _lib as L
from . import probe as LP
from . import runtime as R


def variance_scaling_(tensor: torch.Tensor, scale: float = 1.0, mode: str = "fan_in",
                      distribution: str = "truncated_normal") -> torch.Tensor:
    fan_out, fan_in = tensor.shape[0], int(math.prod(tensor.shape[1:]))
    denom = {"fan_in": fan_in, "fan_out": fan_out, "fan_avg": (fan_in + fan_out) / 2}[mode]
    variance = scale / denom
    with torch.no_grad():
        if distribution == "truncated_normal":
            std = math.sqrt(variance) / 0.87962566103423978
            nn.init.trunc_normal_(tensor, std=std, a=-2 * std, b=2 * std)
        elif distribution == "normal":
            tensor.normal_(std=math.sqrt(variance))
        elif distribution == "uniform":
            bound = math.sqrt(3 * variance)
            tensor.uniform_(-bound, bound)
        else:
            raise ValueError(f"invalid distribution {distribution}")
    return tensor


def lecun_normal_(tensor: torch.Tensor) -> torch.Tensor:
    return variance_scaling_(tensor, mode="fan_in", distribution="truncated_normal")


def make_cross_attention_mask(query_mask: torch.Tensor, kv_mask: torch.Tensor) -> torch.Tensor:
    batch_size, query_len = query_mask.shape
    _, key_len = kv_mask.shape
    mask = query_mask[:, :, None] & kv_mask[:, None, :] if query_mask.dtype == torch.bool and \
        kv_mask.dtype == torch.bool else torch.einsum("bi,bj->bij", (query_mask, kv_mask))
    assert mask.shape == (batch_size, query_len, key_len)
    return mask


FUSED_SELF_HEADS = {(128, 128), (64, 64), (32, 32), (32, 160)}


def _no_training_dropout(mod: nn.Module, *probs: float) -> None:
    if mod.training and any(p > 0.0 for p in probs):
        raise NotImplementedError("the HIP path is forward/inference only: call .eval() or use dropout_prob=0")


class _HipModule(nn.Module):

    def __init__(self):
        super().__init__()
        self._pio_cache = None
        self._pio_block_cache = None

    def _cached(self, key, builder):
        c = self._pio_cache
        if c is None or c[0] != key:
            desc, keep = builder()
            self._pio_cache = c = (key, desc, keep)
        return c[1]

    def _apply(self, fn, *a, **k):
        self._pio_cache = self._pio_block_cache = None
        return super()._apply(fn, *a, **k)

    def _load_from_state_dict(self, *a, **k):
        self._pio_cache = self._pio_block_cache = None
        return super()._load_from_state_dict(*a, **k)


class Attention(_HipModule):

    def __init__(self, q_in_channels: int, k_in_channels: int = None, v_in_channels: int = None,
                 num_heads: int = 8, init_scale: float = 1.0, with_final_bias: bool = True,
                 final_init_scale_multiplier: float = 1., dropout_prob: float = 0.0,
                 qk_out_channels: int = None, v_out_channels: int = None, output_channels: int = None):
        super().__init__()
        self._num_heads = num_heads
        final_init_scale = final_init_scale_multiplier * init_scale
        if qk_out_channels is None:
            qk_out_channels = q_in_channels
        if v_out_channels is None:
            v_out_channels = qk_out_channels
        if output_channels is None:
            output_channels = v_out_channels
        self._qk_channels_per_head = qk_out_channels // num_heads
        self._v_channels_per_head = v_out_channels // num_heads
        if qk_out_channels % num_heads != 0:
            raise ValueError(f"qk_out_channels ({qk_out_channels}) must be divisible by"
                             f" num_heads ({num_heads}).")
        if v_out_channels % num_heads != 0:
            raise ValueError(f"v_channels ({v_out_channels}) must be divisible by"
                             f" num_heads ({num_heads}).")
        self.proj_q = nn.Linear(q_in_channels, qk_out_channels, bias=True)
        self.proj_k = nn.Linear(k_in_channels, qk_out_channels, bias=True)
        self.proj_v = nn.Linear(v_in_channels, v_out_channels, bias=True)
        for lin in (self.proj_q, self.proj_k, self.proj_v):
            variance_scaling_(lin.weight, scale=init_scale, mode="fan_in", distribution="truncated_normal")
            nn.init.constant_(lin.bias, 0)
        self.dropout = nn.Dropout(dropout_prob)
        self.final = nn.Linear(v_out_channels, output_channels, bias=with_final_bias)
        variance_scaling_(self.final.weight, scale=final_init_scale, mode="fan_in",
                          distribution="truncated_normal")
        if self.final.bias is not None:
            nn.init.constant_(self.final.bias, 0)

    def _build_desc(self, ov=None):
        dtype, wlevel, split = R.policy_dtype()
        H = self._num_heads
        two = wlevel >= 3
        wt = (lambda lin: ov[lin]) if ov else (lambda lin: lin.weight)
        q = R.PackedLinear(wt(self.proj_q), self.proj_q.bias, H, 1, dtype, two)
        k = R.PackedLinear(wt(self.proj_k), self.proj_k.bias, H, 1, dtype, two)
        fine = R.policy_fine_split()
        v_two, o_two = wlevel >= 1 or "proj_v" in fine, wlevel >= 1 or "final" in fine
        v = R.PackedLinear(wt(self.proj_v), self.proj_v.bias, H, 1, dtype, v_two)
        o = R.PackedLinear(wt(self.final), self.final.bias, 1, H, dtype, o_two, k_channels=False)
        dk, dv = self._qk_channels_per_head, self._v_channels_per_head
        d = L.Attention(q.desc, k.desc, v.desc, o.desc, H, dk, dv, R.pad8(dk), R.pad8(dv),
                        self.proj_q.in_features, self.proj_k.in_features, self.proj_v.in_features,
                        self.final.out_features, dtype, R.attention_act_split())
        keep = [q, k, v, o]
        kin = self.proj_k.in_features
        if H == 1 and kin == self.proj_v.in_features and dk == kin and dv == kin and (
                wlevel == 0 or os.environ.get("PIO_KV_FOLD_ANY") == "1"):
            with torch.no_grad():
                Wk, Wv, Wo = wt(self.proj_k).double(), wt(self.proj_v).double(), wt(self.final).double()
                bv = self.proj_v.bias.double() if self.proj_v.bias is not None else torch.zeros(kin, device=Wv.device)
                bo = self.final.bias.double() if self.final.bias is not None else 0.0
                kq = R.PackedLinear(Wk.t().float().contiguous(), None, 1, 1, dtype, True, k_channels=False)
                vo = R.PackedLinear((Wo @ Wv).float().contiguous(), (Wo @ bv + bo).float().contiguous(), 1, 1, dtype,
                                    True, k_channels=False)
            d.kq, d.vo = kq.desc, vo.desc
            keep += [kq, vo]
        if self.proj_q.in_features == self.proj_k.in_features and not split:
            qk = R.PackedStack([(wt(self.proj_q), self.proj_q.bias), (wt(self.proj_k), self.proj_k.bias)],
                               H, dtype, two)
            d.qk = qk.desc
            keep.append(qk)
            if (wlevel <= 2 and not two and self.proj_v.in_features == self.proj_q.in_features
                    and (R.pad8(dk), R.pad8(dv)) in FUSED_SELF_HEADS
                    and (not v_two or (2 * H * R.pad8(dk)) % 256 == 0)):
                qkv = R.PackedStack([(wt(self.proj_q), self.proj_q.bias), (wt(self.proj_k), self.proj_k.bias),
                                     (wt(self.proj_v), self.proj_v.bias)], H, dtype, [False, False, v_two])
                d.qkv = qkv.desc
                keep.append(qkv)
        return d, keep

    def _params(self):
        return (self.proj_q.weight, self.proj_q.bias, self.proj_k.weight, self.proj_k.bias, self.proj_v.weight,
                self.proj_v.bias, self.final.weight, self.final.bias)

    def _desc(self) -> L.Attention:
        return self._cached(R.param_key(*self._params()), self._build_desc)

    def forward(self, inputs_q, inputs_k, inputs_v, attention_mask=None, attention_bias=None,
                return_matrix=False):
        if R.cpu_plumbing(inputs_q, "Attention.forward"):
            from . import cpu_plumbing as CP
            return CP.attention(self, inputs_q, inputs_k, inputs_v, attention_mask, attention_bias, return_matrix)
        R.require_device(inputs_q, "Attention.forward")
        _no_training_dropout(self, self.dropout.p)
        lib = L.lib()
        xq, xk, xv = R.as_f32_3d(inputs_q), R.as_f32_3d(inputs_k), R.as_f32_3d(inputs_v)
        if inputs_v is inputs_k:
            xv = xk
        B, Tq, _ = xq.shape
        Tk = xk.shape[1]
        dev = xq.device
        d = self._desc()
        H = self._num_heads
        fm, fm_ptr = R.mask_u8(attention_mask, (B, Tq, Tk), dev)
        bias_t = None
        if attention_bias is not None:
            bias_t = torch.broadcast_to(attention_bias.to(device=dev, dtype=torch.float32),
                                        (B, H, Tq, Tk)).contiguous()
        out = torch.empty((B, Tq, self.final.out_features), dtype=torch.float32, device=dev)
        probs = torch.empty((B, H, Tq, Tk), dtype=torch.float32, device=dev) if return_matrix else None
        nbytes = lib.pio_attention_workspace_bytes(d, B, Tq, Tk)
        ws = R.workspace(dev, nbytes)
        tq, tk, tv = R.tensor3(xq), R.tensor3(xk), R.tensor3(xv)
        LP.expect("attention")
        with R.on_device(dev):
            L.check(lib.pio_attention_fwd(d, tq, tk, tv, None, None, fm_ptr,
                                          bias_t.data_ptr() if bias_t is not None else None, out.data_ptr(),
                                          probs.data_ptr() if probs is not None else None, ws.data_ptr(),
                                          ws.numel(), R.stream_ptr(dev)), "pio_attention_fwd")
        out = R.forward_only(out, inputs_q, inputs_k, inputs_v, *self._params())
        if return_matrix:
            return probs, out
        return out


class MLP(_HipModule):

    def __init__(self, in_channels: int, out_channels: int = None, widening_factor: int = 4,
                 dropout_prob: float = 0.0, init_scale: float = 1.):
        super().__init__()
        out_channels = out_channels or in_channels
        self.fc1 = nn.Linear(in_channels, widening_factor * in_channels)
        variance_scaling_(self.fc1.weight, scale=init_scale, mode="fan_in", distribution="truncated_normal")
        nn.init.constant_(self.fc1.bias, 0)
        self.fc2 = nn.Linear(widening_factor * in_channels, out_channels)
        variance_scaling_(self.fc2.weight, scale=init_scale, mode="fan_in", distribution="truncated_normal")
        nn.init.constant_(self.fc2.bias, 0)
        self.dropout = nn.Dropout(dropout_prob)

    def _build_desc(self, ov=None):
        dtype, wlevel, split = R.policy_dtype()
        two = wlevel >= 2
        fine = R.policy_fine_split()
        wt = (lambda lin: ov[lin]) if ov else (lambda lin: lin.weight)
        f1 = R.PackedLinear(wt(self.fc1), self.fc1.bias, 1, 1, dtype, two or "fc1" in fine, n_channels=True)
        f2 = R.PackedLinear(wt(self.fc2), self.fc2.bias, 1, 1, dtype, two or "fc2" in fine)
        d = L.Mlp(f1.desc, f2.desc, self.fc1.in_features, self.fc1.out_features, self.fc2.out_features, dtype,
                  int(split))
        return d, [f1, f2]

    def _params(self):
        return (self.fc1.weight, self.fc1.bias, self.fc2.weight, self.fc2.bias)

    def _desc(self) -> L.Mlp:
        return self._cached(R.param_key(*self._params()), self._build_desc)

    def forward(self, x):
        if R.cpu_plumbing(x, "MLP.forward"):
            from . import cpu_plumbing as CP
            return CP.mlp(self, x)
        R.require_device(x, "MLP.forward")
        _no_training_dropout(self, self.dropout.p)
        lib = L.lib()
        shape = x.shape
        x3 = R.as_f32_3d(x.reshape(-1, shape[-2], shape[-1]) if x.dim() != 3 else x)
        d = self._desc()
        dev = x3.device
        out = torch.empty(x3.shape[:2] + (self.fc2.out_features,), dtype=torch.float32, device=dev)
        rows = x3.shape[0] * x3.shape[1]
        ws = R.workspace(dev, lib.pio_mlp_workspace_bytes(d, rows))
        with R.on_device(dev):
            L.check(lib.pio_mlp_fwd(d, R.tensor3(x3), out.data_ptr(), ws.data_ptr(), ws.numel(), R.stream_ptr(dev)),
                    "pio_mlp_fwd")
        out = R.forward_only(out, x, *self._params())
        return out.reshape(shape[:-1] + (self.fc2.out_features,))


class SelfAttention(_HipModule):

    def __init__(self, in_channels: int, widening_factor: int = 4, dropout_prob: float = 0.0,
                 dropout_attn_prob: float = 0.0, num_heads: int = 8, att_init_scale: float = 1.0,
                 dense_init_scale: float = 1.0, qk_channels: int = None, v_channels: int = None):
        super().__init__()
        if qk_channels is None:
            qk_channels = in_channels
        if v_channels is None:
            v_channels = qk_channels
        self.mlp = MLP(in_channels=v_channels, widening_factor=widening_factor, dropout_prob=dropout_prob,
                       init_scale=dense_init_scale)
        self.attention = Attention(q_in_channels=in_channels, k_in_channels=in_channels,
                                   v_in_channels=in_channels, num_heads=num_heads, init_scale=att_init_scale,
                                   qk_out_channels=qk_channels, v_out_channels=v_channels,
                                   dropout_prob=dropout_attn_prob)
        self.layer_norm1 = nn.LayerNorm(in_channels)
        self.layer_norm2 = nn.LayerNorm(v_channels)
        self.dropout = nn.Dropout(dropout_prob)
        self._in_channels = in_channels
        self._v_channels = v_channels

    def _build_desc(self):
        keep = []
        a = self.attention._desc()
        m = self.mlp._desc()
        d = L.SelfAttention(R.layernorm_desc(self.layer_norm1, keep), R.layernorm_desc(self.layer_norm2, keep), a, m)
        self._build_ln_fold(d, a, keep)
        return d, keep + [self.attention._pio_cache, self.mlp._pio_cache]

    def _desc_blocks(self, nblk: int):
        key = R.param_key(*self._params()) + (nblk,)
        c = self._pio_block_cache
        if c is None or c[0] != key:
            dtype, _wlevel, _split = R.policy_dtype()
            att, mlp = self.attention, self.mlp
            lins = (att.proj_q, att.proj_k, att.proj_v, att.final, mlp.fc1, mlp.fc2)
            descs, keep = [], []
            with torch.no_grad():
                g1, g2 = self.layer_norm1.weight.float(), self.layer_norm2.weight.float()
                plain = {lin: R.feedback_images(lin.weight, nblk, dtype) for lin in lins}
                fold = {lin: R.feedback_images(lin.weight.float() * g[None, :], nblk, dtype)
                        for lin, g in ((att.proj_q, g1), (att.proj_k, g1), (att.proj_v, g1), (mlp.fc1, g2))}
                for b in range(nblk):
                    a, ka = att._build_desc({lin: plain[lin][b] for lin in lins[:4]})
                    m, km = mlp._build_desc({lin: plain[lin][b] for lin in lins[4:]})
                    d = L.SelfAttention(R.layernorm_desc(self.layer_norm1, keep), R.layernorm_desc(self.layer_norm2, keep),
                                        a, m)
                    self._build_ln_fold(d, a, keep, {lin: imgs[b] for lin, imgs in fold.items()})
                    descs.append(d)
                    keep.extend([ka, km])
            self._pio_block_cache = c = (key, descs, keep)
        return c[1]

    def _build_ln_fold(self, d, a, keep, fold_ov=None):
        dtype, wlevel, split = R.policy_dtype()
        att, mlp = self.attention, self.mlp
        C_ = self._in_channels
        if (wlevel > 2 or split or C_ % 256 or not 512 <= C_ <= 1536 or not a.qkv.w_hi
                or mlp.fc1.in_features != C_ or mlp.fc1.out_features != C_ or att.proj_q.in_features != C_):
            return
        with torch.no_grad():
            g1, b1 = self.layer_norm1.weight.float(), self.layer_norm1.bias.float()
            g2, b2 = self.layer_norm2.weight.float(), self.layer_norm2.bias.float()

            def folded(lin, g, b):
                w = lin.weight.float()
                bias = lin.bias.float() if lin.bias is not None else torch.zeros(w.shape[0], device=w.device)
                wg = fold_ov[lin] if fold_ov else w * g[None, :]
                return wg.contiguous(), (w @ b + bias).contiguous()

            H = att._num_heads
            qkv = R.PackedStack([folded(att.proj_q, g1, b1), folded(att.proj_k, g1, b1), folded(att.proj_v, g1, b1)],
                                H, dtype, [False, False, wlevel >= 1 or "proj_v" in R.policy_fine_split()])
            fc1 = R.PackedLinear(*folded(mlp.fc1, g2, b2), 1, 1, dtype, wlevel >= 2, n_channels=True)
            qkv_c = (qkv.hi.float() + (qkv.lo.float() if qkv.lo is not None else 0)).sum(1).contiguous()
            fc1_c = (fc1.hi.float() + (fc1.lo.float() if fc1.lo is not None else 0)).sum(1).contiguous()
        d.fold = L.LnFold(qkv.desc, qkv_c.data_ptr(), fc1.desc, fc1_c.data_ptr())
        keep.extend([qkv, fc1, qkv_c, fc1_c])

    def _params(self):
        return self.attention._params() + self.mlp._params() + (self.layer_norm1.weight, self.layer_norm1.bias,
                                                                 self.layer_norm2.weight, self.layer_norm2.bias)

    def _desc(self) -> L.SelfAttention:
        return self._cached(R.param_key(*self._params()), self._build_desc)

    def forward(self, inputs, *, attention_mask=None, attention_bias=None, return_matrix: bool = False):
        if R.cpu_plumbing(inputs, "SelfAttention.forward"):
            from . import cpu_plumbing as CP
            if self._v_channels != self._in_channels:
                raise RuntimeError(f"The size of tensor a ({self._in_channels}) must match the size of tensor b "
                                   f"({self._v_channels}) at non-singleton dimension 2")
            return CP.self_attention(self, inputs, attention_mask, attention_bias, return_matrix)
        R.require_device(inputs, "SelfAttention.forward")
        _no_training_dropout(self, self.dropout.p, self.attention.dropout.p, self.mlp.dropout.p)
        if self._v_channels != self._in_channels:
            raise RuntimeError(f"The size of tensor a ({self._in_channels}) must match the size of tensor b "
                               f"({self._v_channels}) at non-singleton dimension 2")
        lib = L.lib()
        x = R.as_f32_3d(inputs)
        B, N, D = x.shape
        dev = x.device
        H = self.attention._num_heads
        d = self._desc()
        fm, fm_ptr = R.mask_u8(attention_mask, (B, N, N), dev)
        bias_t = None
        if attention_bias is not None:
            bias_t = torch.broadcast_to(attention_bias.to(device=dev, dtype=torch.float32), (B, H, N, N)).contiguous()
        out = torch.empty((B, N, D), dtype=torch.float32, device=dev)
        probs = torch.empty((B, H, N, N), dtype=torch.float32, device=dev) if return_matrix else None
        ws = R.workspace(dev, lib.pio_self_attention_workspace_bytes(d, B, N))
        LP.expect("attention")
        with R.on_device(dev):
            L.check(lib.pio_self_attention_fwd(d, R.tensor3(x), None, None, fm_ptr,
                                               bias_t.data_ptr() if bias_t is not None else None, out.data_ptr(),
                                               probs.data_ptr() if probs is not None else None, ws.data_ptr(),
                                               ws.numel(), R.stream_ptr(dev)), "pio_self_attention_fwd")
        out = R.forward_only(out, inputs, *self._params())
        if return_matrix:
            return probs, out
        return out


class CrossAttention(_HipModule):

    def __init__(self, q_in_channels: int, kv_in_channels: int, widening_factor: int = 1,
                 dropout_prob: float = 0.0, dropout_attn_prob: float = 0.0, num_heads: int = 8,
                 attn_init_scale: float = 1.0, mlp_init_scale: float = 1.0, shape_for_attn: str = "kv",
                 use_query_residual: bool = True, qk_channels: int = None, v_channels: int = None):
        super().__init__()
        self._use_query_residual = use_query_residual
        output_channels = q_in_channels
        if qk_channels is None:
            if shape_for_attn == "q":
                qk_channels = q_in_channels
            elif shape_for_attn == "kv":
                qk_channels = kv_in_channels
            else:
                raise ValueError(f"Unknown value {shape_for_attn} for "
                                 "shape_for_attention.")
        if v_channels is None:
            v_channels = qk_channels
        self.attention = Attention(q_in_channels=q_in_channels, k_in_channels=kv_in_channels,
                                   v_in_channels=kv_in_channels, num_heads=num_heads, init_scale=attn_init_scale,
                                   dropout_prob=dropout_attn_prob, qk_out_channels=qk_channels,
                                   v_out_channels=v_channels, output_channels=output_channels)
        self.mlp = MLP(in_channels=output_channels, widening_factor=widening_factor, dropout_prob=dropout_prob,
                       init_scale=mlp_init_scale)
        self.layer_norm_q = nn.LayerNorm(q_in_channels)
        self.layer_norm_kv = nn.LayerNorm(kv_in_channels)
        self.layer_norm2 = nn.LayerNorm(output_channels)
        self.dropout = nn.Dropout(dropout_prob)

    def _build_desc(self):
        keep = []
        d = L.CrossAttention(R.layernorm_desc(self.layer_norm_q, keep), R.layernorm_desc(self.layer_norm_kv, keep),
                             R.layernorm_desc(self.layer_norm2, keep), self.attention._desc(), self.mlp._desc(),
                             1 if self._use_query_residual else 0)
        return d, keep + [self.attention._pio_cache, self.mlp._pio_cache]

    def _params(self):
        return self.attention._params() + self.mlp._params() + (
            self.layer_norm_q.weight, self.layer_norm_q.bias, self.layer_norm_kv.weight, self.layer_norm_kv.bias,
            self.layer_norm2.weight, self.layer_norm2.bias)

    def _desc(self) -> L.CrossAttention:
        return self._cached(R.param_key(*self._params()), self._build_desc)

    def forward(self, inputs_q, inputs_kv, *, attention_mask=None, attention_bias=None,
                return_matrix: bool = False):
        if R.cpu_plumbing(inputs_q, "CrossAttention.forward"):
            from . import cpu_plumbing as CP
            return CP.cross_attention(self, inputs_q, inputs_kv, attention_mask, attention_bias, return_matrix)
        R.require_device(inputs_q, "CrossAttention.forward")
        _no_training_dropout(self, self.dropout.p, self.attention.dropout.p, self.mlp.dropout.p)
        lib = L.lib()
        xq, xkv = R.as_f32_3d(inputs_q), R.as_f32_3d(inputs_kv)
        B, Tq, Cq = xq.shape
        Tk = xkv.shape[1]
        dev = xq.device
        H = self.attention._num_heads
        d = self._desc()
        fm, fm_ptr = R.mask_u8(attention_mask, (B, Tq, Tk), dev)
        bias_t = None
        if attention_bias is not None:
            bias_t = torch.broadcast_to(attention_bias.to(device=dev, dtype=torch.float32),
                                        (B, H, Tq, Tk)).contiguous()
        out = torch.empty((B, Tq, Cq), dtype=torch.float32, device=dev)
        probs = torch.empty((B, H, Tq, Tk), dtype=torch.float32, device=dev) if return_matrix else None
        ws = R.workspace(dev, lib.pio_cross_attention_workspace_bytes(d, B, Tq, Tk))
        LP.expect("attention")
        with R.on_device(dev):
            L.check(lib.pio_cross_attention_fwd(d, R.tensor3(xq), R.tensor3(xkv), None, None, fm_ptr,
                                                bias_t.data_ptr() if bias_t is not None else None, out.data_ptr(),
                                                probs.data_ptr() if probs is not None else None, ws.data_ptr(),
                                                ws.numel(), R.stream_ptr(dev)), "pio_cross_attention_fwd")
        out = R.forward_only(out, inputs_q, inputs_kv, *self._params())
        if return_matrix:
            return probs, out
        return out
```

Baseline: 1982 samples/s.

## Precompute layer-normed query projections for learned latent and decoder query tables

Adds kernels that pack the LayerNorm plus Q projection of the parameter-only query tables, for the encoder latents and the decoder output queries. An optional K-folded variant is also packed for the KV-fold cross-attention route. The packs are cached per module and keyed on parameter versions, and new qpack entry points let the cross-attention skip the per-step query cast and Q GEMM. The cost is extra cached buffers and invalidation logic. Capture fails if the pack is stale, so one eager forward is required after any parameter write.

```diff
diff --git a/include/pio_hip.h b/include/pio_hip.h
--- a/include/pio_hip.h
+++ b/include/pio_hip.h
@@ -133,6 +133,20 @@
 int pio_pack_linear(const float *w, const float *bias, int32_t out, int32_t in, int64_t ldw,
                     int32_t row_heads, int32_t col_heads, void *dst_hi, void *dst_lo, float *dst_bias,
                     int32_t dst_row0, int32_t k_pad, int32_t dtype, void *stream);
+
+size_t pio_query_pack_bytes(int32_t Tq, int32_t width);
+size_t pio_query_pack_workspace_bytes(int32_t Tq, int32_t nq);
+int pio_pack_projected_query(const float *table, int64_t ld, int32_t Tq, int32_t D, const float *gamma, const float *beta,
+                             float eps, const float *wq, const float *bq, int32_t nq, int32_t heads, int32_t dtype,
+                             void *q_hi, void *q_lo, void *workspace, size_t workspace_bytes, void *stream);
+int pio_pack_folded_query(const float *table, int64_t ld, int32_t Tq, int32_t D, const float *gamma, const float *beta,
+                          float eps, const float *wq, const float *bq, int32_t nq, const float *wk, int32_t kin,
+                          int32_t dtype, void *qf_hi, void *qf_lo, void *workspace, size_t workspace_bytes, void *stream);
+
+typedef struct pio_query_pack_t {
+    const void *q_hi, *q_lo;
+    const void *qf_hi, *qf_lo;
+} pio_query_pack_t;
 
 int pio_layernorm_cast(const pio_tensor3_t *x, const pio_layernorm_t *ln, void *y, void *y_lo, int32_t c_pad,
                        int32_t dtype, void *stream);
@@ -262,6 +276,20 @@
                           const pio_tensor3_t *query, const pio_tensor3_t *query_tail, const pio_tensor3_t *latents,
                           const uint8_t *query_mask, float *out, void *workspace, size_t workspace_bytes, void *stream);
 
+int pio_cross_attention_fwd_qpack(const pio_cross_attention_t *c, const pio_tensor3_t *inputs_q,
+                                  const pio_tensor3_t *inputs_kv, const uint8_t *kv_mask, const uint8_t *q_mask,
+                                  const uint8_t *full_mask, const float *attention_bias, float *out, float *probs_out,
+                                  void *workspace, size_t workspace_bytes, void *stream, const pio_query_pack_t *qp);
+int pio_encoder_fwd_qpack(const pio_cross_attention_t *cross, const pio_self_attention_t *layers, int32_t L,
+                          int32_t num_blocks, int32_t per_block, const pio_tensor3_t *inputs,
+                          const pio_tensor3_t *inputs_tail, const pio_tensor3_t *latents, const uint8_t *input_mask,
+                          float *out, void *workspace, size_t workspace_bytes, void *stream,
+                          const pio_call_opts_t *opts, const pio_query_pack_t *qp);
+int pio_decoder_fwd_qpack(const pio_cross_attention_t *cross, const pio_linear_t *final_layer, int32_t final_out,
+                          const pio_tensor3_t *query, const pio_tensor3_t *latents, const uint8_t *query_mask,
+                          float *out, void *workspace, size_t workspace_bytes, void *stream,
+                          const pio_query_pack_t *qp);
+
 #ifdef __cplusplus
 }
 #endif
diff --git a/perceiverio_pytorch_amd/_lib.py b/perceiverio_pytorch_amd/_lib.py
--- a/perceiverio_pytorch_amd/_lib.py
+++ b/perceiverio_pytorch_amd/_lib.py
@@ -64,6 +64,10 @@
     _fields_ = [("ln_fold", C.c_int32), ("cu_budget", C.c_int32)]
 
 
+class QueryPack(C.Structure):
+    _fields_ = [("q_hi", C.c_void_p), ("q_lo", C.c_void_p), ("qf_hi", C.c_void_p), ("qf_lo", C.c_void_p)]
+
+
 class Gemm(C.Structure):
     _fields_ = [("A", C.c_void_p), ("B", C.c_void_p), ("A_lo", C.c_void_p), ("B_lo", C.c_void_p), ("C", C.c_void_p),
                 ("C_lo", C.c_void_p),
@@ -107,6 +111,12 @@
     "pio_set_cu_budget": (C.c_int, [_i32]),
     "pio_packed_weight_bytes": (_sz, [_i32, _i32, _i32, _i32]),
     "pio_pack_linear": (C.c_int, [_vp, _vp, _i32, _i32, _i64, _i32, _i32, _vp, _vp, _vp, _i32, _i32, _i32, _vp]),
+    "pio_query_pack_bytes": (_sz, [_i32, _i32]),
+    "pio_query_pack_workspace_bytes": (_sz, [_i32, _i32]),
+    "pio_pack_projected_query": (C.c_int, [_vp, _i64, _i32, _i32, _vp, _vp, _f, _vp, _vp, _i32, _i32, _i32, _vp, _vp, _vp,
+                                           _sz, _vp]),
+    "pio_pack_folded_query": (C.c_int, [_vp, _i64, _i32, _i32, _vp, _vp, _f, _vp, _vp, _i32, _vp, _i32, _i32, _vp, _vp, _vp,
+                                        _sz, _vp]),
     "pio_layernorm_cast": (C.c_int, [P(Tensor3), P(LayerNorm), _vp, _vp, _i32, _i32, _vp]),
     "pio_layernorm_cast_cat": (C.c_int, [P(Tensor3), P(Tensor3), P(LayerNorm), _vp, _vp, _i32, _i32, _vp]),
     "pio_bn_relu_maxpool_tokens": (C.c_int, [_vp, _vp, _vp, _vp, _i32, _i32, _i32, _i32, _i32, _i32, _vp]),
@@ -147,6 +157,12 @@
                                          _vp, _vp, _vp, _i32]),
     "pio_decoder_fwd_split": (C.c_int, [P(CrossAttention), P(Linear), _i32, P(Tensor3), P(Tensor3), P(Tensor3), _vp, _vp, _vp,
                                         _sz, _vp]),
+    "pio_cross_attention_fwd_qpack": (C.c_int, [P(CrossAttention), P(Tensor3), P(Tensor3), _vp, _vp, _vp, _vp, _vp, _vp,
+                                                _vp, _sz, _vp, P(QueryPack)]),
+    "pio_encoder_fwd_qpack": (C.c_int, [P(CrossAttention), P(SelfAttention), _i32, _i32, _i32, P(Tensor3), P(Tensor3),
+                                        P(Tensor3), _vp, _vp, _vp, _sz, _vp, P(CallOpts), P(QueryPack)]),
+    "pio_decoder_fwd_qpack": (C.c_int, [P(CrossAttention), P(Linear), _i32, P(Tensor3), P(Tensor3), _vp, _vp, _vp, _sz,
+                                        _vp, P(QueryPack)]),
 }
 
 _lib = None
diff --git a/perceiverio_pytorch_amd/csrc/pio_blocks.hip b/perceiverio_pytorch_amd/csrc/pio_blocks.hip
--- a/perceiverio_pytorch_amd/csrc/pio_blocks.hip
+++ b/perceiverio_pytorch_amd/csrc/pio_blocks.hip
@@ -188,6 +188,7 @@
 struct QCache {
     Pair pair;
     bool valid;
+    bool packed = false, folded = false;
 };
 
 static int materialised_core(const pio_attention_t &a, const AttnOperands &t, bool q_bcast, int B, int Tq, int Tk,
@@ -275,7 +276,9 @@
                           const LnFold *fold_out = nullptr, int64_t out_ld = 0, const QCache *qc = nullptr) {
     if (!out_ld) out_ld = a.out;
     PIO_TRY(check_attention(a));
-    if (qc) {
+    const bool q_folded = qc && qc->folded;
+    if (q_folded && !qc->pair.hi) return PIO_E_ARG;
+    if (qc && !q_folded) {
         if (!qc->pair.hi || (a.act_split && !qc->pair.lo)) return PIO_E_ARG;
         w.q16 = qc->pair;
     }
@@ -286,7 +289,7 @@
     call.B = B; call.Bq = Bq; call.Tq = Tq; call.Tk = Tk; call.q_bcast = q_bcast; call.same_qk = xq.hi == xk.hi;
     call.same_kv = xk.hi == xv.hi; call.kv_fold_on = kv_fold_enabled();
     call.kv_mask = kv_mask; call.q_mask = q_mask; call.full_mask = full_mask; call.bias = attention_bias;
-    call.probs = probs_out; call.qcache = qc; call.fold_in = fold_in; call.fold_out = fold_out;
+    call.probs = probs_out; call.qcache = qc && !q_folded; call.fold_in = fold_in; call.fold_out = fold_out;
     call.fold_qkv = (fold_in && fold_in->in_part) ? fold_in->w : nullptr;
     call.qkv_adjacent = (char *)w.q16.hi < (char *)w.k16.hi && (char *)w.k16.hi < (char *)w.vt16.hi &&
                         (size_t)((char *)w.vt16.hi - (char *)w.q16.hi) + (size_t)B * ldo * tkv * 2 >= (size_t)B * Tq * ld3 * 2;
@@ -296,6 +299,7 @@
     if (r.qk_pair && (!w.q16.lo || !w.k16.lo)) return PIO_E_ARG;
     if (r.need_scores && !w.scores) return PIO_E_WORKSPACE;
     const bool kv_fold = r.core == AttnCore::KVFOLD_XATTN || r.core == AttnCore::KVFOLD_XTALL;
+    if (q_folded && !kv_fold) return PIO_E_ARG;
     const int64_t sQ = q_bcast ? 0 : 1;
 
     AttnOperands t = {};
@@ -310,12 +314,15 @@
         t.sQb = t.sKb = t.sVb = (int64_t)Tq * ld3; t.sOb = (int64_t)Tq * ldo;
     } else if (kv_fold) {
         const int64_t kvp = a.dkp, ldx = padc(a.k_in);
-        PIO_TRY(linear_fwd(a.q, a.dtype, xq, (int64_t)Bq * Tq, w.q16.hi, w.q16.lo, false, 0, hdk, 0, nullptr, s));
-        PIO_RANGE(PIO_RK_Q, a.dtype, w.q16.hi, (int64_t)Bq * Tq, hdk, hdk, 1, 0, s);
-        PIO_TRY(linear_fwd(a.kq, a.dtype, w.q16, (int64_t)Bq * Tq, w.k16.hi, w.k16.lo, false, 0, kvp, 0, nullptr, s));
-        PIO_RANGE(PIO_RK_Q, a.dtype, w.k16.hi, (int64_t)Bq * Tq, kvp, kvp, 1, 0, s);
+        if (!q_folded) {
+            PIO_TRY(linear_fwd(a.q, a.dtype, xq, (int64_t)Bq * Tq, w.q16.hi, w.q16.lo, false, 0, hdk, 0, nullptr, s));
+            PIO_RANGE(PIO_RK_Q, a.dtype, w.q16.hi, (int64_t)Bq * Tq, hdk, hdk, 1, 0, s);
+            PIO_TRY(linear_fwd(a.kq, a.dtype, w.q16, (int64_t)Bq * Tq, w.k16.hi, w.k16.lo, false, 0, kvp, 0, nullptr, s));
+        }
+        const void *qf = q_folded ? qc->pair.hi : w.k16.hi;
+        PIO_RANGE(PIO_RK_Q, a.dtype, qf, (int64_t)Bq * Tq, kvp, kvp, 1, 0, s);
         PIO_TRY(transpose16_launch(xk.hi, ldx, B, Tk, (int)kvp, w.vt16.hi, tkv, s));
-        t.Q = w.k16.hi; t.K = xk.hi; t.VT = w.vt16.hi;
+        t.Q = qf; t.K = xk.hi; t.VT = w.vt16.hi;
         t.ldq = kvp; t.ldk = ldx; t.ldvt = tkv; t.ldo = kvp;
         t.sQb = sQ * Tq * kvp; t.sKb = (int64_t)Tk * ldx; t.sVb = kvp * tkv; t.sOb = (int64_t)Tq * kvp;
     } else {
@@ -326,6 +333,8 @@
         } else {
             if (!(qc && qc->valid)) {
                 PIO_TRY(linear_fwd(a.q, a.dtype, xq, (int64_t)Bq * Tq, w.q16.hi, w.q16.lo, false, 0, ldq, 0, nullptr, s));
+                PIO_RANGE(PIO_RK_Q, a.dtype, w.q16.hi, (int64_t)Bq * Tq, ldq, ldq, 1, 0, s);
+            } else if (qc->packed) {
                 PIO_RANGE(PIO_RK_Q, a.dtype, w.q16.hi, (int64_t)Bq * Tq, ldq, ldq, 1, 0, s);
             }
             PIO_TRY(linear_fwd(a.k, a.dtype, xk, (int64_t)B * Tk, w.k16.hi, w.k16.lo, false, 0, ldq, 0, nullptr, s));
@@ -619,12 +628,25 @@
     }
 };
 
+static int query_pack_form(const pio_attention_t &a, const pio_query_pack_t &qp, int B, int Bq, int Tq, int Tk, bool q_bcast,
+                           const uint8_t *kv_mask, const uint8_t *q_mask, const uint8_t *full_mask, const float *bias,
+                           const float *probs) {
+    if (qp.qf_hi) {
+        AttnCall c = {};
+        c.B = B; c.Bq = Bq; c.Tq = Tq; c.Tk = Tk; c.q_bcast = q_bcast; c.same_kv = true; c.kv_fold_on = kv_fold_enabled();
+        c.kv_mask = kv_mask; c.q_mask = q_mask; c.full_mask = full_mask; c.bias = bias; c.probs = probs;
+        const AttnRoute r = attn_route(a, c);
+        if (r.err == PIO_OK && (r.core == AttnCore::KVFOLD_XATTN || r.core == AttnCore::KVFOLD_XTALL)) return 2;
+    }
+    return (qp.q_hi && (!a.act_split || qp.q_lo)) ? 1 : 0;
+}
+
 static int cross_attention_run(const pio_cross_attention_t &ca, const pio_tensor3_t &iq, const pio_tensor3_t &ikv,
                                const uint8_t *kv_mask, const uint8_t *q_mask, const uint8_t *full_mask,
                                const float *attention_bias, float *out, float *probs_out, CrossPlan &p,
                                hipStream_t s, const pio_tensor3_t *ikv_tail = nullptr, int64_t out_ld = 0,
                                const QCache *qc = nullptr, const Pair *out16 = nullptr,
-                               const pio_tensor3_t *iq_tail = nullptr) {
+                               const pio_tensor3_t *iq_tail = nullptr, const pio_query_pack_t *qp = nullptr) {
     const int B = iq.B, Tq = iq.T, Tk = ikv.T;
     const int64_t rows = (int64_t)B * Tq;
     const int kv_c = ikv.C + (ikv_tail ? ikv_tail->C : 0);
@@ -640,10 +662,25 @@
     const pio_tensor3_t q1 = p.q_bcast ? first_batch(iq) : iq;
     const Pair qa = pair_if(p.q16, ca.attn.act_split);
     if (qc && ca.use_query_residual) return PIO_E_ARG;
+    QCache packed_q{};
+    if (qp) {
+        if (qc || iq_tail || !(p.q_bcast || B == 1)) return PIO_E_ARG;
+        if (((uintptr_t)qp->q_hi | (uintptr_t)qp->q_lo | (uintptr_t)qp->qf_hi | (uintptr_t)qp->qf_lo) & 15) return PIO_E_ALIGN;
+        const int form = query_pack_form(ca.attn, *qp, B, p.q_bcast ? 1 : B, Tq, Tk, p.q_bcast, kv_mask, q_mask, full_mask,
+                                         attention_bias, probs_out);
+        if (form) {
+            packed_q.pair.hi = const_cast<void *>(form == 2 ? qp->qf_hi : qp->q_hi);
+            packed_q.pair.lo = const_cast<void *>(form == 2 ? qp->qf_lo : qp->q_lo);
+            packed_q.valid = packed_q.packed = true;
+            packed_q.folded = form == 2;
+            qc = &packed_q;
+        }
+    }
     if (iq_tail) {
         PIO_TRY(layernorm_cast_cat_launch(iq, *iq_tail, ca.ln_q, qa.hi, qa.lo, padc(q_c), ca.attn.dtype, s));
         PIO_RANGE(PIO_RK_CAST, ca.attn.dtype, qa.hi, rows, q_c, padc(q_c), 1, 0, s);
-    } else if (!(qc && qc->valid)) PIO_TRY(cast_pair(q1, &ca.ln_q, qa, padc(q_c), ca.attn.dtype, s));
+    } else if (!(qc && qc->valid) || (qc->packed && range_probe_active()))
+        PIO_TRY(cast_pair(q1, &ca.ln_q, qa, padc(q_c), ca.attn.dtype, s));
     const Residual rq = residual_of(iq);
     PIO_TRY(attention_core(ca.attn, qa, p.q_bcast, p.kv16, p.kv16, B, Tq, Tk, kv_mask, q_mask, full_mask,
                            attention_bias, ca.use_query_residual ? &rq : nullptr, p.x1, probs_out, p.core, s, nullptr,
@@ -780,12 +817,20 @@
                             const uint8_t *kv_mask, const uint8_t *q_mask, const uint8_t *full_mask,
                             const float *attention_bias, float *out, float *probs_out, void *workspace,
                             size_t workspace_bytes, void *stream) {
+    return pio_cross_attention_fwd_qpack(ca, iq, ikv, kv_mask, q_mask, full_mask, attention_bias, out, probs_out, workspace,
+                                         workspace_bytes, stream, nullptr);
+}
+
+int pio_cross_attention_fwd_qpack(const pio_cross_attention_t *ca, const pio_tensor3_t *iq, const pio_tensor3_t *ikv,
+                                  const uint8_t *kv_mask, const uint8_t *q_mask, const uint8_t *full_mask,
+                                  const float *attention_bias, float *out, float *probs_out, void *workspace,
+                                  size_t workspace_bytes, void *stream, const pio_query_pack_t *qp) {
     if (!ca || !iq || !ikv || !out || !workspace) return PIO_E_ARG;
     CrossPlan p;
     const bool qb = (iq->stride_b == 0 && iq->B > 1);
     if (p.carve(workspace, *ca, iq->B, iq->T, ikv->T, qb) > workspace_bytes) return PIO_E_WORKSPACE;
     return cross_attention_run(*ca, *iq, *ikv, kv_mask, q_mask, full_mask, attention_bias, out, probs_out, p,
-                               (hipStream_t)stream);
+                               (hipStream_t)stream, nullptr, 0, nullptr, nullptr, nullptr, qp);
 }
 
 size_t pio_encoder_workspace_bytes(const pio_cross_attention_t *cross, const pio_self_attention_t *layers, int32_t L,
@@ -829,6 +874,15 @@
                          const pio_tensor3_t *inputs_tail, const pio_tensor3_t *latents, const uint8_t *input_mask,
                          float *out, void *workspace, size_t workspace_bytes, void *stream,
                          const pio_call_opts_t *opts) {
+    return pio_encoder_fwd_qpack(cross, layers, L, num_blocks, per_block, inputs, inputs_tail, latents, input_mask, out,
+                                 workspace, workspace_bytes, stream, opts, nullptr);
+}
+
+int pio_encoder_fwd_qpack(const pio_cross_attention_t *cross, const pio_self_attention_t *layers, int32_t L,
+                          int32_t num_blocks, int32_t per_block, const pio_tensor3_t *inputs,
+                          const pio_tensor3_t *inputs_tail, const pio_tensor3_t *latents, const uint8_t *input_mask,
+                          float *out, void *workspace, size_t workspace_bytes, void *stream,
+                          const pio_call_opts_t *opts, const pio_query_pack_t *qp) {
     if (!cross || !inputs || !latents || !out || !workspace || (L > 0 && !layers)) return PIO_E_ARG;
     CallOpts scope(opts);
     if (L < 0 || num_blocks < 0) return PIO_E_SHAPE;
@@ -842,7 +896,7 @@
         const bool qb = (latents->stride_b == 0 && B > 1);
         cp.carve(workspace, *cross, B, N, M, qb, true);
         PIO_TRY(cross_attention_run(*cross, *latents, *inputs, input_mask, nullptr, nullptr, nullptr, out, nullptr,
-                                    cp, s, inputs_tail));
+                                    cp, s, inputs_tail, 0, nullptr, nullptr, nullptr, qp));
     }
     const pio_tensor3_t z = {out, (int64_t)N * D, D, B, N, D};
     range_part.set(PIO_RP_STACK);
@@ -881,7 +935,7 @@
 static int decoder_run(const pio_cross_attention_t *cross, const pio_linear_t *final_layer, int32_t final_out,
                        const pio_tensor3_t *query, const pio_tensor3_t *query_tail, const pio_tensor3_t *latents,
                        const uint8_t *query_mask, float *out, void *workspace, size_t workspace_bytes, void *stream,
-                       void *q16_hi, void *q16_lo, int32_t q16_valid) {
+                       void *q16_hi, void *q16_lo, int32_t q16_valid, const pio_query_pack_t *qp = nullptr) {
     if (!cross || !query || !latents || !out || !workspace) return PIO_E_ARG;
     const int q_c = query->C + (query_tail ? query_tail->C : 0);
     QCache qcache{{q16_hi, q16_lo}, q16_valid != 0};
@@ -901,7 +955,7 @@
     }();
     const bool direct = final_layer && y16_direct && final_layer->k == padc(q_c);
     PIO_TRY(cross_attention_run(*cross, *query, *latents, nullptr, query_mask, nullptr, nullptr, y, nullptr, p.cp,
-                                s, nullptr, y_ld, qc, direct ? &p.y16 : nullptr, query_tail));
+                                s, nullptr, y_ld, qc, direct ? &p.y16 : nullptr, query_tail, qp));
     if (!final_layer) return PIO_OK;
     if (final_layer->k != padc(q_c)) return PIO_E_SHAPE;
     const pio_tensor3_t ty = {y, (int64_t)Q * y_ld, y_ld, B, Q, q_c};
@@ -918,6 +972,14 @@
                        workspace_bytes, stream, q16_hi, q16_lo, q16_valid);
 }
 
+int pio_decoder_fwd_qpack(const pio_cross_attention_t *cross, const pio_linear_t *final_layer, int32_t final_out,
+                          const pio_tensor3_t *query, const pio_tensor3_t *latents, const uint8_t *query_mask,
+                          float *out, void *workspace, size_t workspace_bytes, void *stream,
+                          const pio_query_pack_t *qp) {
+    return decoder_run(cross, final_layer, final_out, query, nullptr, latents, query_mask, out, workspace,
+                       workspace_bytes, stream, nullptr, nullptr, 0, qp);
+}
+
 int pio_decoder_fwd_split(const pio_cross_attention_t *cross, const pio_linear_t *final_layer, int32_t final_out,
                           const pio_tensor3_t *query, const pio_tensor3_t *query_tail, const pio_tensor3_t *latents,
                           const uint8_t *query_mask, float *out, void *workspace, size_t workspace_bytes, void *stream) {
diff --git a/perceiverio_pytorch_amd/csrc/pio_qpack.hip b/perceiverio_pytorch_amd/csrc/pio_qpack.hip
--- /dev/null
+++ b/perceiverio_pytorch_amd/csrc/pio_qpack.hip
@@ -0,0 +1,150 @@
+#include "pio_internal.h"
+
+namespace pio {
+
+static __device__ __forceinline__ float f32_round_odd(double v) {
+    const float f = (float)v;
+    const double d = (double)f;
+    if (d == v || !(fabs(v) <= 3.0e38)) return f;
+    uint32_t u = __float_as_uint(f);
+    if (fabs(d) > fabs(v)) u -= 1;
+    return __uint_as_float(u | 1u);
+}
+
+template <int DT>
+static __device__ __forceinline__ void store_pair(double v, typename Op<DT>::T *hi, typename Op<DT>::T *lo, int64_t o) {
+    const typename Op<DT>::T h = Op<DT>::from_f32(f32_round_odd(v));
+    hi[o] = h;
+    if (lo) lo[o] = Op<DT>::from_f32(f32_round_odd(v - (double)Op<DT>::to_f32(h)));
+}
+
+__global__ void qpack_stats_kernel(const float *__restrict__ x, int64_t ld, int Tq, int D, double eps,
+                                   double *__restrict__ stats) {
+    const int t = blockIdx.x * blockDim.x + threadIdx.x;
+    if (t >= Tq) return;
+    const float *row = x + (int64_t)t * ld;
+    double sum = 0.0;
+    for (int d = 0; d < D; ++d) sum += (double)row[d];
+    const double mean = sum / D;
+    double sq = 0.0;
+    for (int d = 0; d < D; ++d) {
+        const double c = (double)row[d] - mean;
+        sq += c * c;
+    }
+    stats[2 * t] = mean;
+    stats[2 * t + 1] = 1.0 / sqrt(sq / D + eps);
+}
+
+__global__ void qpack_project_kernel(const float *__restrict__ x, int64_t ld, int Tq, int D,
+                                     const float *__restrict__ gamma, const float *__restrict__ beta,
+                                     const double *__restrict__ stats, const float *__restrict__ wq,
+                                     const float *__restrict__ bq, int nq, double *__restrict__ q64) {
+    const int64_t idx = (int64_t)blockIdx.x * blockDim.x + threadIdx.x;
+    if (idx >= (int64_t)Tq * nq) return;
+    const int t = (int)(idx / nq), n = (int)(idx % nq);
+    const float *row = x + (int64_t)t * ld, *w = wq + (int64_t)n * D;
+    const double mean = stats[2 * t], rstd = stats[2 * t + 1];
+    double acc = 0.0;
+    for (int d = 0; d < D; ++d)
+        acc += (((double)row[d] - mean) * rstd * (double)gamma[d] + (double)beta[d]) * (double)w[d];
+    q64[idx] = acc + (bq ? (double)bq[n] : 0.0);
+}
+
+template <int DT>
+__global__ void qpack_store_kernel(const double *__restrict__ q64, int Tq, int nq, int dk, int dkp, int heads,
+                                   typename Op<DT>::T *hi, typename Op<DT>::T *lo) {
+    const int64_t idx = (int64_t)blockIdx.x * blockDim.x + threadIdx.x;
+    const int width = heads * dkp;
+    if (idx >= (int64_t)Tq * width) return;
+    const int t = (int)(idx / width), c = (int)(idx % width), h = c / dkp, j = c % dkp;
+    store_pair<DT>(j < dk ? q64[(int64_t)t * nq + h * dk + j] : 0.0, hi, lo, idx);
+}
+
+template <int DT>
+__global__ void qpack_fold_kernel(const double *__restrict__ q64, int Tq, int nq, const float *__restrict__ wk, int kin,
+                                  int kvp, typename Op<DT>::T *hi, typename Op<DT>::T *lo) {
+    const int64_t idx = (int64_t)blockIdx.x * blockDim.x + threadIdx.x;
+    if (idx >= (int64_t)Tq * kvp) return;
+    const int t = (int)(idx / kvp), j = (int)(idx % kvp);
+    double acc = 0.0;
+    if (j < kin) {
+        const double *q = q64 + (int64_t)t * nq;
+        for (int n = 0; n < nq; ++n) acc += q[n] * (double)wk[(int64_t)n * kin + j];
+    }
+    store_pair<DT>(acc, hi, lo, idx);
+}
+
+static size_t qpack_workspace(int Tq, int nq) {
+    return (size_t)round_up((int64_t)Tq * 2 * 8, 256) + (size_t)round_up((int64_t)Tq * nq * 8, 256);
+}
+
+static int query_pack_launch(const float *table, int64_t ld, int Tq, int D, const float *gamma, const float *beta,
+                             float eps, const float *wq, const float *bq, int nq, int heads, const float *wk, int kin,
+                             int dtype, void *hi, void *lo, void *workspace, size_t workspace_bytes, hipStream_t s) {
+    if (!table || !gamma || !beta || !wq || !hi || !workspace) return PIO_E_ARG;
+    if (dtype != PIO_DT_F16 && dtype != PIO_DT_BF16) return PIO_E_ARG;
+    if (Tq <= 0 || D <= 0 || nq <= 0 || heads <= 0 || (nq % heads) || ld < D || (wk && (kin <= 0 || heads != 1)))
+        return PIO_E_SHAPE;
+    if (((uintptr_t)hi & 1) || ((uintptr_t)lo & 1) || ((uintptr_t)workspace & 7)) return PIO_E_ALIGN;
+    if (qpack_workspace(Tq, nq) > workspace_bytes) return PIO_E_WORKSPACE;
+    Carver c(workspace);
+    double *stats = (double *)c.take((size_t)Tq * 2 * 8);
+    double *q64 = (double *)c.take((size_t)Tq * nq * 8);
+    const int dk = nq / heads, dkp = pad8(dk), kvp = pad8(kin);
+    const int64_t n_out = (int64_t)Tq * (wk ? kvp : heads * dkp);
+    ProfScope prof(PROF_PACK, 2.0 * Tq * nq * ((double)D + (wk ? kin : 0)), 4.0 * ((double)Tq * D + (double)nq * D), s);
+    const int th = 256;
+    const auto blocks = [](int64_t n) { return dim3((unsigned)((n + 255) / 256)); };
+    hipLaunchKernelGGL(qpack_stats_kernel, blocks(Tq), dim3(th), 0, s, table, ld, Tq, D, (double)eps, stats);
+    hipLaunchKernelGGL(qpack_project_kernel, blocks((int64_t)Tq * nq), dim3(th), 0, s, table, ld, Tq, D, gamma, beta,
+                       stats, wq, bq, nq, q64);
+    if (wk) {
+        if (dtype == PIO_DT_F16)
+            hipLaunchKernelGGL((qpack_fold_kernel<PIO_DT_F16>), blocks(n_out), dim3(th), 0, s, q64, Tq, nq, wk, kin, kvp,
+                               (_Float16 *)hi, (_Float16 *)lo);
+        else
+            hipLaunchKernelGGL((qpack_fold_kernel<PIO_DT_BF16>), blocks(n_out), dim3(th), 0, s, q64, Tq, nq, wk, kin, kvp,
+                               (__bf16 *)hi, (__bf16 *)lo);
+    } else {
+        if (dtype == PIO_DT_F16)
+            hipLaunchKernelGGL((qpack_store_kernel<PIO_DT_F16>), blocks(n_out), dim3(th), 0, s, q64, Tq, nq, dk, dkp, heads,
+                               (_Float16 *)hi, (_Float16 *)lo);
+        else
+            hipLaunchKernelGGL((qpack_store_kernel<PIO_DT_BF16>), blocks(n_out), dim3(th), 0, s, q64, Tq, nq, dk, dkp,
+                               heads, (__bf16 *)hi, (__bf16 *)lo);
+    }
+    return launch_status();
+}
+
+}
+
+using namespace pio;
+
+extern "C" {
+
+size_t pio_query_pack_bytes(int32_t Tq, int32_t width) {
+    if (Tq <= 0 || width <= 0) return 0;
+    return (size_t)round_up((int64_t)Tq * pad8(width) * 2, 256);
+}
+
+size_t pio_query_pack_workspace_bytes(int32_t Tq, int32_t nq) {
+    if (Tq <= 0 || nq <= 0) return 0;
+    return qpack_workspace(Tq, nq);
+}
+
+int pio_pack_projected_query(const float *table, int64_t ld, int32_t Tq, int32_t D, const float *gamma, const float *beta,
+                             float eps, const float *wq, const float *bq, int32_t nq, int32_t heads, int32_t dtype,
+                             void *q_hi, void *q_lo, void *workspace, size_t workspace_bytes, void *stream) {
+    return query_pack_launch(table, ld, Tq, D, gamma, beta, eps, wq, bq, nq, heads, nullptr, 0, dtype, q_hi, q_lo,
+                             workspace, workspace_bytes, (hipStream_t)stream);
+}
+
+int pio_pack_folded_query(const float *table, int64_t ld, int32_t Tq, int32_t D, const float *gamma, const float *beta,
+                          float eps, const float *wq, const float *bq, int32_t nq, const float *wk, int32_t kin,
+                          int32_t dtype, void *qf_hi, void *qf_lo, void *workspace, size_t workspace_bytes, void *stream) {
+    if (!wk) return PIO_E_ARG;
+    return query_pack_launch(table, ld, Tq, D, gamma, beta, eps, wq, bq, nq, 1, wk, kin, dtype, qf_hi, qf_lo, workspace,
+                             workspace_bytes, (hipStream_t)stream);
+}
+
+}
diff --git a/perceiverio_pytorch_amd/perceiver.py b/perceiverio_pytorch_amd/perceiver.py
--- a/perceiverio_pytorch_amd/perceiver.py
+++ b/perceiverio_pytorch_amd/perceiver.py
@@ -66,6 +66,9 @@
         dev = x.device
         with R.precision(self.cross_attend_policy):
             cross = self.cross_attend._desc()
+            qpack = self.cross_attend._query_pack(z0, self.latent_pos_enc.pos_embs, "PerceiverEncoder.forward")
+            if qpack is not None:
+                cross = self.cross_attend._desc_packed_q()
         Lyr = len(self.self_attends)
         per_block = R.policy_block_feedback() and self._num_blocks > 1 and Lyr > 0
         nset = self._num_blocks if per_block else 1
@@ -100,9 +103,9 @@
             LP.mark_range("cross")
             try:
                 with R.on_device(dev):
-                    L.check(lib.pio_encoder_fwd_opts(cross, layers, Lyr, self._num_blocks, int(per_block), R.tensor3(x),
-                                                     tail3, R.tensor3(z0), im_ptr, out.data_ptr(), ws.data_ptr(),
-                                                     ws.numel(), R.stream_ptr(dev), opts), "pio_encoder_fwd")
+                    L.check(lib.pio_encoder_fwd_qpack(cross, layers, Lyr, self._num_blocks, int(per_block), R.tensor3(x),
+                                                      tail3, R.tensor3(z0), im_ptr, out.data_ptr(), ws.data_ptr(),
+                                                      ws.numel(), R.stream_ptr(dev), opts, qpack), "pio_encoder_fwd")
             finally:
                 LP.mark_range("attention")
             return self._finish(out, flag, inputs, inputs_tail, latents, input_mask)
@@ -121,9 +124,10 @@
                     xs, zs = x[i * bs:(i + 1) * bs], z0[i * bs:(i + 1) * bs]
                     ws = R.workspace(dev, lib.pio_encoder_workspace_bytes(cross, layers, Lyr, bs, M, N))
                     mp = im_ptr + i * bs * M if im_ptr is not None else None
-                    L.check(lib.pio_encoder_fwd_opts(cross, layers, Lyr, self._num_blocks, 0, R.tensor3(xs), None,
-                                                     R.tensor3(zs), mp, out[i * bs:(i + 1) * bs].data_ptr(),
-                                                     ws.data_ptr(), ws.numel(), side.cuda_stream, opts), "pio_encoder_fwd")
+                    L.check(lib.pio_encoder_fwd_qpack(cross, layers, Lyr, self._num_blocks, 0, R.tensor3(xs), None,
+                                                      R.tensor3(zs), mp, out[i * bs:(i + 1) * bs].data_ptr(),
+                                                      ws.data_ptr(), ws.numel(), side.cuda_stream, opts, qpack),
+                            "pio_encoder_fwd")
             finally:
                 LP.mark_range("attention")
         for side in sides:
@@ -204,7 +208,7 @@
             self._final_cache = (key, R.PackedLinear(self.final_layer.weight, self.final_layer.bias, 1, 1, dtype, two))
         return self._final_cache[1]
 
-    def forward(self, query, latents, *, query_mask=None, q_cache=None):
+    def forward(self, query, latents, *, query_mask=None, q_cache=None, query_table=None):
         query_tail = None
         if isinstance(query, (tuple, list)):
             query, query_tail = query
@@ -233,6 +237,11 @@
         ws = R.workspace(dev, lib.pio_decoder_workspace_bytes(cross, fin_ptr, B, Q, N))
         qhi = qlo = None
         valid = 0
+        qpack = None
+        if query_table is not None and q_cache is None and query_tail is None:
+            qpack = self.decoding_cross_attn._query_pack(q, query_table, "PerceiverDecoder.forward")
+            if qpack is not None:
+                cross = self.decoding_cross_attn._desc_packed_q()
         if q_cache is not None and not self._use_query_residual and query_tail is None:
             ca = self.decoding_cross_attn
             Bq = 1 if (q.stride(0) == 0 and B > 1) else B
@@ -261,6 +270,10 @@
                     L.check(lib.pio_decoder_fwd_split(cross, fin_ptr, out_ch, R.tensor3(q), R.tensor3(query_tail),
                                                       R.tensor3(z), qm_ptr, out.data_ptr(), ws.data_ptr(), ws.numel(),
                                                       R.stream_ptr(dev)), "pio_decoder_fwd_split")
+                elif qpack is not None:
+                    L.check(lib.pio_decoder_fwd_qpack(cross, fin_ptr, out_ch, R.tensor3(q), R.tensor3(z), qm_ptr,
+                                                      out.data_ptr(), ws.data_ptr(), ws.numel(), R.stream_ptr(dev), qpack),
+                            "pio_decoder_fwd")
                 else:
                     L.check(lib.pio_decoder_fwd_qcache(cross, fin_ptr, out_ch, R.tensor3(q), R.tensor3(z), qm_ptr,
                                                        out.data_ptr(), ws.data_ptr(), ws.numel(), R.stream_ptr(dev), qhi,
@@ -412,6 +425,16 @@
         return (getattr(q, "_position_encoding", 0) is None and getattr(q, "_concat_preprocessed_input", False)
                 and not self._decoder._use_query_residual and self.decoder_query_rows is None
                 and q.n_query_channels() == self.query_channels)
+
+    def _query_table(self):
+        qs = list(self._output_queries.values())
+        if len(qs) != 1:
+            return None
+        enc = getattr(qs[0], "_position_encoding", None)
+        if (isinstance(enc, TrainablePositionEncoding) and not getattr(qs[0], "_concat_preprocessed_input", False)
+                and qs[0].n_query_channels() == self.query_channels):
+            return enc.pos_embs
+        return None
 
     def decoder_query(self, inputs, modality_sizes, inputs_without_pos=None, subsampled_points=None):
         per_mod = restructure(modality_sizes, inputs)
@@ -492,7 +515,7 @@
                 from .dist import decode_query_sharded
                 outputs = decode_query_sharded(self._decoder, query, latents, query_mask, *query_shard)
             else:
-                outputs = self._decoder(query, latents, query_mask=query_mask)
+                outputs = self._decoder(query, latents, query_mask=query_mask, query_table=self._query_table())
         if self._output_postprocessors:
             per_mod = restructure(query_sizes, outputs)
             with R.precision(self.decoder_policy):
diff --git a/perceiverio_pytorch_amd/runtime.py b/perceiverio_pytorch_amd/runtime.py
--- a/perceiverio_pytorch_amd/runtime.py
+++ b/perceiverio_pytorch_amd/runtime.py
@@ -405,12 +405,46 @@
 
 def invalidate_packed_weights(module: torch.nn.Module) -> None:
     for m in module.modules():
+        if hasattr(m, "_stale_query_packs"):
+            m._stale_query_packs()
         if hasattr(m, "_pio_cache"):
             m._pio_cache = None
         if hasattr(m, "_pio_block_cache"):
             m._pio_block_cache = None
         if hasattr(m, "_final_cache"):
             m._final_cache = None
+
+
+def query_pack_enabled(what: str = "") -> bool:
+    mode = os.environ.get("PIO_QUERY_PACK", "1")
+    if mode in ("encoder", "decoder"):
+        return what.lower().startswith("perceiver" + mode)
+    return mode != "0"
+
+
+def kv_fold_split_weights() -> bool:
+    return os.environ.get("PIO_KV_FOLD_X2W", "1" if KV_FOLD_X2W_DEFAULT else "0") != "0"
+
+
+KV_FOLD_X2W_DEFAULT = False
+
+
+def table_rows(q: torch.Tensor, table: Optional[torch.Tensor]) -> Optional[int]:
+    if table is None or not isinstance(table, torch.Tensor) or table.dim() != 2 or q.dim() != 3:
+        return None
+    if not (table.is_cuda and q.is_cuda) or table.dtype != torch.float32 or q.dtype != torch.float32:
+        return None
+    if not table.is_contiguous() or table.numel() == 0 or q.numel() == 0:
+        return None
+    B, Tq, D = q.shape
+    if D != table.shape[1] or (B > 1 and q.stride(0) != 0) or (Tq > 1 and q.stride(1) != D) or (D > 1 and q.stride(2) != 1):
+        return None
+    if q.untyped_storage().data_ptr() != table.untyped_storage().data_ptr():
+        return None
+    off = q.data_ptr() - table.data_ptr()
+    if off < 0 or off % (4 * D) or off // (4 * D) + Tq > table.shape[0]:
+        return None
+    return Tq
 
 
 class _ForwardOnly(torch.autograd.Function):
diff --git a/perceiverio_pytorch_amd/transformer_primitives.py b/perceiverio_pytorch_amd/transformer_primitives.py
--- a/perceiverio_pytorch_amd/transformer_primitives.py
+++ b/perceiverio_pytorch_amd/transformer_primitives.py
@@ -128,8 +128,10 @@
                         self.final.out_features, dtype, R.attention_act_split())
         keep = [q, k, v, o]
         kin = self.proj_k.in_features
+        any_policy = os.environ.get("PIO_KV_FOLD_ANY") == "1"
+        with_packed_q = R.get_precision_policy() == "fp16x2w" and R.kv_fold_split_weights() and not ov
         if H == 1 and kin == self.proj_v.in_features and dk == kin and dv == kin and (
-                wlevel == 0 or os.environ.get("PIO_KV_FOLD_ANY") == "1"):
+                wlevel == 0 or any_policy or with_packed_q):
             with torch.no_grad():
                 Wk, Wv, Wo = wt(self.proj_k).double(), wt(self.proj_v).double(), wt(self.final).double()
                 bv = self.proj_v.bias.double() if self.proj_v.bias is not None else torch.zeros(kin, device=Wv.device)
@@ -137,7 +139,10 @@
                 kq = R.PackedLinear(Wk.t().float().contiguous(), None, 1, 1, dtype, True, k_channels=False)
                 vo = R.PackedLinear((Wo @ Wv).float().contiguous(), (Wo @ bv + bo).float().contiguous(), 1, 1, dtype,
                                     True, k_channels=False)
-            d.kq, d.vo = kq.desc, vo.desc
+            if wlevel == 0 or any_policy:
+                d.kq, d.vo = kq.desc, vo.desc
+            else:
+                d._fold_with_packed_q = (kq.desc, vo.desc)
             keep += [kq, vo]
         if self.proj_q.in_features == self.proj_k.in_features and not split:
             qk = R.PackedStack([(wt(self.proj_q), self.proj_q.bias), (wt(self.proj_k), self.proj_k.bias)],
@@ -406,10 +411,83 @@
 
     def _build_desc(self):
         keep = []
+        a = self.attention._desc()
         d = L.CrossAttention(R.layernorm_desc(self.layer_norm_q, keep), R.layernorm_desc(self.layer_norm_kv, keep),
-                             R.layernorm_desc(self.layer_norm2, keep), self.attention._desc(), self.mlp._desc(),
+                             R.layernorm_desc(self.layer_norm2, keep), a, self.mlp._desc(),
                              1 if self._use_query_residual else 0)
+        d._packed_q = d
+        fold = getattr(a, "_fold_with_packed_q", None)
+        if fold is not None:
+            d._packed_q = L.CrossAttention.from_buffer_copy(d)
+            d._packed_q.attn.kq, d._packed_q.attn.vo = fold
         return d, keep + [self.attention._pio_cache, self.mlp._pio_cache]
+
+    def _desc_packed_q(self) -> L.CrossAttention:
+        return self._desc()._packed_q
+
+    def _stale_query_packs(self):
+        for e in (self.__dict__.get("_pio_qpack") or {}).values():
+            e["key"] = None
+
+    def _apply(self, fn, *a, **k):
+        self.__dict__["_pio_qpack"] = None
+        return super()._apply(fn, *a, **k)
+
+    def _load_from_state_dict(self, *a, **k):
+        self._stale_query_packs()
+        return super()._load_from_state_dict(*a, **k)
+
+    def _query_pack(self, q: torch.Tensor, table, what: str) -> Optional[L.QueryPack]:
+        if not R.query_pack_enabled(what) or R.table_rows(q, table) is None:
+            return None
+        att, ln = self.attention, self.layer_norm_q
+        wq, bq, wk = att.proj_q.weight, att.proj_q.bias, att.proj_k.weight
+        params = (table, ln.weight, ln.bias, wq, bq, wk)
+        if any(p is not None and (p.dtype != torch.float32 or not p.is_contiguous() or p.device != q.device)
+               for p in params):
+            return None
+        dev = q.device
+        Tq, D = q.shape[1], q.shape[2]
+        dtype = R.policy_dtype()[0]
+        H, nq, kin = att._num_heads, wq.shape[0], wk.shape[1]
+        key = (R.param_key(*params), q.data_ptr(), Tq)
+        packs = self.__dict__.get("_pio_qpack")
+        if packs is None:
+            packs = self.__dict__["_pio_qpack"] = {}
+        slot = (dtype, q.data_ptr(), Tq, str(dev))
+        e = packs.get(slot)
+        proj = R.attention_act_split() != 0 or os.environ.get("PIO_QUERY_PACK") == "all"
+        if e is not None and e["key"] == key:
+            return e["pack"] if proj else e["pack_folded"]
+        if R.capturing(dev):
+            raise L.PioError(f"{what}: the pack-time queries are missing or stale, and during stream capture a cache is "
+                             "only READ: nothing is allocated or validated inside a graph -- run one eager forward after "
+                             "the last parameter write, then capture")
+        lib = L.lib()
+        fold = H == 1 and kin == att.proj_v.in_features and nq == kin and att.proj_v.out_features == kin
+        if e is None:
+            width = H * R.pad8(nq // H)
+            with torch.inference_mode(False):
+                def image(w):
+                    return torch.empty(lib.pio_query_pack_bytes(Tq, w), dtype=torch.uint8, device=dev)
+                e = {"q": (image(width), image(width)), "qf": (image(kin), image(kin)) if fold else None}
+            e["pack"] = L.QueryPack(e["q"][0].data_ptr(), e["q"][1].data_ptr(),
+                                    e["qf"][0].data_ptr() if fold else None, e["qf"][1].data_ptr() if fold else None)
+            e["pack_folded"] = L.QueryPack(None, None, e["pack"].qf_hi, e["pack"].qf_lo) if fold else None
+            packs[slot] = e
+        nws = lib.pio_query_pack_workspace_bytes(Tq, nq)
+        ws = R.workspace(dev, nws)
+        head = (q.data_ptr(), D, Tq, D, ln.weight.data_ptr(), ln.bias.data_ptr(), float(ln.eps), wq.data_ptr(),
+                bq.data_ptr() if bq is not None else None, nq)
+        with R.on_device(dev):
+            L.check(lib.pio_pack_projected_query(*head, H, dtype, e["q"][0].data_ptr(), e["q"][1].data_ptr(),
+                                                 ws.data_ptr(), ws.numel(), R.stream_ptr(dev)), "pio_pack_projected_query")
+            if fold:
+                L.check(lib.pio_pack_folded_query(*head, wk.data_ptr(), kin, dtype, e["qf"][0].data_ptr(),
+                                                  e["qf"][1].data_ptr(), ws.data_ptr(), ws.numel(), R.stream_ptr(dev)),
+                        "pio_pack_folded_query")
+        e["key"] = key
+        return e["pack"] if proj else e["pack_folded"]
 
     def _params(self):
         return self.attention._params() + self.mlp._params() + (
```

Result: no change. 1988 samples/s, median of 6 (+0.3%).
